# meyerls/FruitNeRF

Measured on AMD Instinct MI355X. Metric: train rays/sec, fruit_nerf on synthetic apple 800x800, higher is better.
Workload: dtype f32 fwd (MLP GEMMs: 3-piece bf16 split, 6 products, ~2^-24) / 2-piece bwd (dX, dW: 3 products, ~2^-17; its forward recompute 3-piece); everything else f32

## Files before the change

### fruitnerf_amd/csrc/hash_scatter.hip

```cpp
#include <stdlib.h>
#include <string.h>

#include "hash_sources.hpp"
#include "sequencer.hpp"

namespace fnr {

constexpr int SC_MAX_ROWS = 8192;
constexpr int SC_MAX_BINS = 256;
constexpr int SC_CHUNK = 512;
constexpr int SC_EMIT_THREADS = 512;
constexpr int SC_PER_THREAD = SC_CHUNK / SC_EMIT_THREADS;
constexpr int SC_BINS_PER_THREAD = 1;
static_assert(SC_MAX_BINS <= SC_EMIT_THREADS, "one bin per thread");
constexpr int SC_CNT_STRIDE = 32;

__device__ unsigned long long g_scatter_overflow_records;
__device__ unsigned long long g_scatter_records[2][64][16];



struct ScatterPlan {
  int log2_rows;
  int bins_per_level;
  long long cap;
  size_t count_bytes, queue_bytes;
  size_t value_bytes;
};

static ScatterPlan scatter_plan(long long N, int n_levels, int log2_T) {
  ScatterPlan p;
  int log2_rows = log2_T - 5;
  if (log2_rows > 13) log2_rows = 13;
  if (log2_rows < 0) log2_rows = 0;
  p.log2_rows = log2_rows;
  p.bins_per_level = 1 << (log2_T - log2_rows);
  const long long avg = (N * 8 + p.bins_per_level - 1) / p.bins_per_level;
  p.cap = (3 * avg + 1023) / 1024 * 1024;
  if (p.cap < 1024) p.cap = 1024;
  const size_t nbins = (size_t)n_levels * p.bins_per_level;
  p.count_bytes = (nbins + 2 * (size_t)n_levels) * SC_CNT_STRIDE * sizeof(unsigned);
  p.value_bytes = nbins * (size_t)p.cap * sizeof(float2);
  p.queue_bytes = p.value_bytes + (nbins * (size_t)p.cap * sizeof(unsigned short) + 255) / 256 * 256;
  return p;
}

__device__ __forceinline__ GridLevel corner_weights(const float (&x)[3], int scaling, uint32_t mask, uint32_t (&h)[8],
                                                    float (&wgt)[8]) {
  GridLevel g = grid_cell(x, scaling);
  grid_corners(g, mask, h);
  const float ox = g.o[0], oy = g.o[1], oz = g.o[2];
  const float mx = 1.0f - ox, my = 1.0f - oy, mz = 1.0f - oz;
  wgt[0] = ox * oy * oz;
  wgt[1] = ox * my * oz;
  wgt[2] = mx * my * oz;
  wgt[3] = mx * oy * oz;
  wgt[4] = ox * oy * mz;
  wgt[5] = ox * my * mz;
  wgt[6] = mx * my * mz;
  wgt[7] = mx * oy * mz;
  return g;
}

template <int CTRL, int ROW_MASK = 0xf>
__device__ __forceinline__ uint32_t dpp_u32(uint32_t old, uint32_t v) {
  return (uint32_t)__builtin_amdgcn_update_dpp((int)old, (int)v, CTRL, ROW_MASK, 0xf, false);
}
template <int CTRL, int ROW_MASK = 0xf>
__device__ __forceinline__ float dpp_f32(float old, float v) {
  return __builtin_bit_cast(float, __builtin_amdgcn_update_dpp(__builtin_bit_cast(int, old), __builtin_bit_cast(int, v),
                                                                 CTRL, ROW_MASK, 0xf, false));
}

struct RunMasks {
  float g1, g2, g4, g8;
  bool tail;
  bool any_run;
};
template <int CTRL>
__device__ __forceinline__ float dpp_shr0_f32(float v) {
  return __builtin_bit_cast(float, __builtin_amdgcn_update_dpp(0, __builtin_bit_cast(int, v), CTRL, 0xf, 0xf, true));
}
__device__ __forceinline__ RunMasks run_structure(uint32_t key_a, uint32_t key_b, int lane) {
  const int j = lane & 15;
  const uint32_t pa = dpp_u32<0x111>(~key_a, key_a), pb = dpp_u32<0x111>(key_b, key_b);
  const bool head = (pa != key_a) || (pb != key_b);
  const unsigned long long heads = __ballot(head);
  const uint32_t row = (uint32_t)(heads >> (lane & 48)) & 0xffffu;
  const uint32_t below = row & ((2u << j) - 1u);
  const int dist = j - (31 - __clz((int)below));
  RunMasks m;
  m.g1 = dist >= 1 ? 1.0f : 0.0f;
  m.g2 = dist >= 2 ? 1.0f : 0.0f;
  m.g4 = dist >= 4 ? 1.0f : 0.0f;
  m.g8 = dist >= 8 ? 1.0f : 0.0f;
  m.tail = (j == 15) || ((row >> (j + 1)) & 1u);
  m.any_run = ~heads != 0ull;
  return m;
}
__device__ __forceinline__ float run_sum(float v, const RunMasks& m) {
  v = fmaf(m.g1, dpp_shr0_f32<0x111>(v), v);
  v = fmaf(m.g2, dpp_shr0_f32<0x112>(v), v);
  v = fmaf(m.g4, dpp_shr0_f32<0x114>(v), v);
  v = fmaf(m.g8, dpp_shr0_f32<0x118>(v), v);
  return v;
}



template <class Source, bool PAIRS>
__global__ __launch_bounds__(SC_EMIT_THREADS) void k_scatter_emit(GridDev grid, Warp warp, Source src, long long N,
                                                      const float2* __restrict__ d_feats, float2* __restrict__ queue_v,
                                                      unsigned short* __restrict__ queue_r, unsigned* __restrict__ qcount, unsigned* __restrict__ qmax,
                                                      long long cap, int log2_rows, int level0, int level_count, int lpb
                                                      ) {
  __shared__ float2 s_val[SC_CHUNK * 8];
  __shared__ unsigned s_key[SC_CHUNK * 8];
  __shared__ unsigned s_cnt[SC_MAX_BINS];
  __shared__ unsigned s_off[SC_MAX_BINS];
  __shared__ unsigned s_base[SC_MAX_BINS];
  __shared__ unsigned s_max;
  __shared__ unsigned s_wsum[SC_EMIT_THREADS / 64];
  const int bins = 1 << (grid.log2_T - log2_rows);
  const int lane = threadIdx.x & 63, wave = threadIdx.x >> 6;
  const uint32_t mask = (1u << grid.log2_T) - 1u;
  const uint32_t row_mask = (1u << log2_rows) - 1u;
  const long long n0 = (long long)blockIdx.x * SC_CHUNK;
  static_assert(SC_PER_THREAD == 1, "one sample per thread");
  const long long n = n0 + threadIdx.x;
  const bool valid = n < N;
  float x[3] = {0.f, 0.f, 0.f};
  float2 gf_next = make_float2(0.f, 0.f);
  const int lrel0 = blockIdx.y * lpb;
  if (valid) {
    gf_next = ntc_load<NT_DFEATS_LD>(&d_feats[(size_t)(level0 + lrel0) * N + n]);
    float px, py, pz;
    src.position(n, px, py, pz);
    warp_position(warp, px, py, pz, x);
  }
  for (int li = 0; li < lpb && lrel0 + li < level_count; ++li) {
  const int lrel = lrel0 + li;
  const int level = level0 + lrel;
  for (int i = threadIdx.x; i < bins; i += SC_EMIT_THREADS) {
    s_cnt[i] = 0;
  }
  if (threadIdx.x == 0) s_max = 0;
  __syncthreads();
  const int scaling = grid.scalings[level];
  const float2 gf = gf_next;
  if (valid && li + 1 < lpb && lrel + 1 < level_count) gf_next = ntc_load<NT_DFEATS_LD>(&d_feats[(size_t)(level + 1) * N + n]);

  uint32_t hk[SC_PER_THREAD][8];
  float vxk[SC_PER_THREAD][8], vyk[SC_PER_THREAD][8];
  float tmax = 0.0f;
  unsigned emit_mask[SC_PER_THREAD];
#pragma unroll
  for (int q = 0; q < SC_PER_THREAD; ++q) {
    float wgt[8];
    const GridLevel g = corner_weights(x, scaling, mask, hk[q], wgt);
    const uint32_t key_a = valid ? (g.f[0] | (g.f[1] << 16)) : 0xffffffffu;
    const uint32_t key_b = valid ? (g.f[2] | ((g.c[0] - g.f[0]) << 16) | ((g.c[1] - g.f[1]) << 17) |
                                    ((g.c[2] - g.f[2]) << 18))
                                 : (0x80000000u | (uint32_t)lane);
    const RunMasks rm = run_structure(key_a, key_b, lane);
    emit_mask[q] = 0;
#pragma unroll
    for (int k = 0; k < 8; ++k) {
      vxk[q][k] = valid ? wgt[k] * gf.x : 0.0f;
      vyk[q][k] = valid ? wgt[k] * gf.y : 0.0f;
    }
    if (rm.any_run) {
#pragma unroll
      for (int k = 0; k < 8; ++k) {
        vxk[q][k] = run_sum(vxk[q][k], rm);
        vyk[q][k] = run_sum(vyk[q][k], rm);
      }
    }
#pragma unroll
    for (int k = 0; k < 8; ++k) {
      if (rm.tail && (vxk[q][k] != 0.0f || vyk[q][k] != 0.0f)) {
        emit_mask[q] |= 1u << k;
        tmax = fmaxf(tmax, fmaxf(fabsf(vxk[q][k]), fabsf(vyk[q][k])));
      }
    }
    if constexpr (PAIRS) {
#pragma unroll
      for (int pr = 0; pr < 4; ++pr) {
        const int ka = (pr == 0) ? 0 : (pr == 1) ? 1 : (pr == 2) ? 4 : 5, kb = (pr == 0) ? 3 : (pr == 1) ? 2 : (pr == 2) ? 7 : 6;
        const unsigned cnt = ((emit_mask[q] >> ka) & 1u) + ((emit_mask[q] >> kb) & 1u);
        if (cnt) atomicAdd(&s_cnt[hk[q][ka] >> log2_rows], cnt);
      }
    } else {
#pragma unroll
      for (int k = 0; k < 8; ++k)
        if ((emit_mask[q] >> k) & 1u) atomicAdd(&s_cnt[hk[q][k] >> log2_rows], 1u);
    }
  }
#pragma unroll
  for (int dsh = 32; dsh >= 1; dsh >>= 1) tmax = fmaxf(tmax, __shfl_xor(tmax, dsh, 64));
  if (lane == 0 && tmax > 0.0f) atomicMax(&s_max, __float_as_uint(tmax));
  __syncthreads();
  if (threadIdx.x == 0 && s_max != 0u) atomicMax(&qmax[(size_t)lrel * SC_CNT_STRIDE], s_max);
  unsigned c4[SC_BINS_PER_THREAD], tsum = 0;
#pragma unroll
  for (int t = 0; t < SC_BINS_PER_THREAD; ++t) {
    const int i = threadIdx.x * SC_BINS_PER_THREAD + t;
    c4[t] = (i < bins) ? s_cnt[i] : 0u;
    tsum += c4[t];
  }
  unsigned incl = tsum;
#pragma unroll
  for (int d = 1; d < 64; d <<= 1) {
    const unsigned u = __shfl_up(incl, d, 64);
    if (lane >= d) incl += u;
  }
  if (lane == 63) s_wsum[wave] = incl;
  __syncthreads();
  unsigned woff = 0;
  for (int w = 0; w < wave; ++w) woff += s_wsum[w];
  unsigned total = 0;
#pragma unroll
  for (int w = 0; w < SC_EMIT_THREADS / 64; ++w) total += s_wsum[w];
  unsigned run = woff + incl - tsum;
#pragma unroll
  for (int t = 0; t < SC_BINS_PER_THREAD; ++t) {
    const int i = threadIdx.x * SC_BINS_PER_THREAD + t;
    if (i < bins) {
      s_off[i] = run;
      s_base[i] = c4[t] ? atomicAdd(&qcount[(size_t)(lrel * bins + i) * SC_CNT_STRIDE], c4[t]) : 0u;
      s_cnt[i] = 0;
      run += c4[t];
    }
  }
  __syncthreads();
#pragma unroll
  for (int q = 0; q < SC_PER_THREAD; ++q) {
    if constexpr (PAIRS) {
#pragma unroll
      for (int pr = 0; pr < 4; ++pr) {
        const int ka = (pr == 0) ? 0 : (pr == 1) ? 1 : (pr == 2) ? 4 : 5, kb = (pr == 0) ? 3 : (pr == 1) ? 2 : (pr == 2) ? 7 : 6;
        const unsigned ea = (emit_mask[q] >> ka) & 1u, eb = (emit_mask[q] >> kb) & 1u;
        if (ea + eb) {
          const unsigned bin = hk[q][ka] >> log2_rows;
          const unsigned pos = s_off[bin] + atomicAdd(&s_cnt[bin], ea + eb);
          if (ea) {
            s_val[pos] = make_float2(vxk[q][ka], vyk[q][ka]);
            s_key[pos] = (hk[q][ka] & row_mask) | (bin << 16);
          }
          if (eb) {
            s_val[pos + ea] = make_float2(vxk[q][kb], vyk[q][kb]);
            s_key[pos + ea] = (hk[q][kb] & row_mask) | (bin << 16);
          }
        }
      }
    } else {
#pragma unroll
      for (int k = 0; k < 8; ++k) {
        if ((emit_mask[q] >> k) & 1u) {
          const int bin = hk[q][k] >> log2_rows;
          const unsigned pos = s_off[bin] + atomicAdd(&s_cnt[bin], 1u);
          s_val[pos] = make_float2(vxk[q][k], vyk[q][k]);
          s_key[pos] = (hk[q][k] & row_mask) | ((unsigned)bin << 16);
        }
      }
    }
  }
  __syncthreads();
  float* table = reinterpret_cast<float*>(grid.table + ((size_t)level << grid.log2_T));
  unsigned overflowed_here = 0;
  for (unsigned i = threadIdx.x; i < total; i += SC_EMIT_THREADS) {
    const float2 v = s_val[i];
    const unsigned key = s_key[i];
    const unsigned bin = key >> 16, row_in_bin = key & 0xffffu;
    const unsigned slot = s_base[bin] + (i - s_off[bin]);
    if ((long long)slot < cap) {
      const size_t q = ((size_t)lrel * bins + bin) * cap + slot;
      queue_v[q] = v;
      queue_r[q] = (unsigned short)row_in_bin;
    } else {
      qmax[(size_t)lrel * SC_CNT_STRIDE + 1] = 1u;
      ++overflowed_here;
      const size_t row = ((size_t)bin << log2_rows) + row_in_bin;
      atomicAdd(table + 2 * row, v.x);
      atomicAdd(table + 2 * row + 1, v.y);
    }
  }
  if (overflowed_here) atomicAdd(&g_scatter_overflow_records, (unsigned long long)overflowed_here);
  __syncthreads();
  }
}

__device__ __forceinline__ void acc_record(unsigned long long* __restrict__ s_acc, unsigned row, const float2& v,
                                           double scale) {
  const long long ix = __double2ll_rn((double)v.x * scale), iy = __double2ll_rn((double)v.y * scale);
  atomicAdd(&s_acc[2 * row], (unsigned long long)ix);
  atomicAdd(&s_acc[2 * row + 1], (unsigned long long)iy);
}

struct AccArgs {
  GridDev grid;
  const float2* queue_v;
  const unsigned short* queue_r;
  unsigned *qcount, *qmax, *qdone;
  long long cap;
  int log2_rows, level0, nbins;
  int kind;
  TableAdam adam;
};

template <bool ADAM>
__device__ __forceinline__ void accumulate_bin(const AccArgs& A, int vblock, unsigned long long* __restrict__ s_acc) {
  const GridDev& grid = A.grid;
  const float2* __restrict__ queue_v = A.queue_v;
  const unsigned short* __restrict__ queue_r = A.queue_r;
  unsigned* __restrict__ qcount = A.qcount;
  unsigned* __restrict__ qmax = A.qmax;
  unsigned* __restrict__ qdone = A.qdone;
  const long long cap = A.cap;
  const int log2_rows = A.log2_rows, level0 = A.level0;
  const TableAdam& adam = A.adam;
  const int rows = 1 << log2_rows;
  const int bins = 1 << (grid.log2_T - log2_rows);
  const int gbin = A.nbins - 1 - vblock;
  const int lrel = gbin / bins, bin = gbin - lrel * bins;
  const int level = level0 + lrel;
  long long n = qcount[(size_t)gbin * SC_CNT_STRIDE];
  const float vmax = __uint_as_float(qmax[(size_t)lrel * SC_CNT_STRIDE]);
  const bool overflowed = qmax[(size_t)lrel * SC_CNT_STRIDE + 1] != 0u;
  {
    const unsigned held_n = (unsigned)n, held_max = __float_as_uint(vmax), held_ovf = overflowed ? 1u : 0u;
    asm volatile("s_waitcnt vmcnt(0) lgkmcnt(0)" ::"v"(held_n), "v"(held_max), "v"(held_ovf) : "memory");
  }
  __syncthreads();
  if (threadIdx.x == 0) {
    qcount[(size_t)gbin * SC_CNT_STRIDE] = 0u;
    if (atomicAdd(&qdone[(size_t)lrel * SC_CNT_STRIDE], 1u) == (unsigned)bins - 1u) {
      qmax[(size_t)lrel * SC_CNT_STRIDE] = 0u;
      qmax[(size_t)lrel * SC_CNT_STRIDE + 1] = 0u;
      qdone[(size_t)lrel * SC_CNT_STRIDE] = 0u;
    }
  }
  const bool have = n != 0 && vmax > 0.0f;
  if (threadIdx.x == 0 && n > 0)
    atomicAdd(&g_scatter_records[A.kind & 1][vblock & 63][0], (unsigned long long)(n > cap ? cap : n));
  if (!ADAM && !have) return;
  if (n > cap) n = cap;
  if (n < 1) n = 1;
  int e;
  (void)frexpf(vmax, &e);
  const int nb = 64 - __clzll((unsigned long long)n);
  int S = 62 - nb - e;
  if (S > 1000) S = 1000;
  const double scale = ldexp(1.0, S), inv = ldexp(1.0, -S);
  for (int i = threadIdx.x; i < 2 * rows; i += blockDim.x) s_acc[i] = 0ull;
  __syncthreads();
  if (!have) n = 0;
  const float2* qv = queue_v + (size_t)gbin * cap;
  const unsigned short* qr = queue_r + (size_t)gbin * cap;
  const float4* qv2 = reinterpret_cast<const float4*>(qv);
  const ushort2* qr2 = reinterpret_cast<const ushort2*>(qr);
  const long long np = n >> 1;
  long long i = threadIdx.x;
  for (; i + 3 * (long long)blockDim.x < np; i += 4 * (long long)blockDim.x) {
    float4 v[4];
    ushort2 row[4];
#pragma unroll
    for (int u = 0; u < 4; ++u) {
      v[u] = ntc_load<NT_QUEUE_LD>(&qv2[i + u * (long long)blockDim.x]);
      row[u] = ntc_load<NT_QUEUE_LD>(&qr2[i + u * (long long)blockDim.x]);
    }
#pragma unroll
    for (int u = 0; u < 4; ++u) {
      acc_record(s_acc, row[u].x, make_float2(v[u].x, v[u].y), scale);
      acc_record(s_acc, row[u].y, make_float2(v[u].z, v[u].w), scale);
    }
  }
  for (; i < np; i += blockDim.x) {
    const float4 v = ntc_load<NT_QUEUE_LD>(&qv2[i]);
    const ushort2 row = ntc_load<NT_QUEUE_LD>(&qr2[i]);
    acc_record(s_acc, row.x, make_float2(v.x, v.y), scale);
    acc_record(s_acc, row.y, make_float2(v.z, v.w), scale);
  }
  if ((n & 1) && threadIdx.x == 0) {
    acc_record(s_acc, qr[n - 1], qv[n - 1], scale);
  }
  __syncthreads();
  float2* dst = grid.table + ((size_t)level << grid.log2_T) + (size_t)bin * rows;
  if constexpr (ADAM) {
    const size_t row0 = ((size_t)level << grid.log2_T) + (size_t)bin * rows;
    const bool wide = rows >= 2 && (((uintptr_t)(adam.p + row0) | (uintptr_t)(adam.m + row0) | (uintptr_t)(adam.v + row0)) & 15u) == 0 &&
                      !overflowed;
    if (wide) {
      float4* P4 = reinterpret_cast<float4*>(adam.p + row0);
      float4* M4 = reinterpret_cast<float4*>(adam.m + row0);
      float4* V4 = reinterpret_cast<float4*>(adam.v + row0);
      unsigned* tw = (adam.touched && rows >= 64) ? adam.touched + (row0 >> 6) : nullptr;
      for (int e4 = threadIdx.x; e4 < (rows >> 1); e4 += blockDim.x) {
        const long long a0 = (long long)s_acc[4 * e4], a1 = (long long)s_acc[4 * e4 + 1],
                        a2 = (long long)s_acc[4 * e4 + 2], a3 = (long long)s_acc[4 * e4 + 3];
        if (tw) {
          const bool now = (a0 | a1 | a2 | a3) != 0;
          const bool ever = (tw[e4 >> 5] >> (e4 & 31)) & 1u;
          if (!now && !ever) continue;
          if (!ever) atomicOr(&tw[e4 >> 5], 1u << (e4 & 31));
        }
        float4 P = P4[e4], M = ntc_load<NT_MOMENT_LD>(&M4[e4]), V = ntc_load<NT_MOMENT_LD>(&V4[e4]);
        const float g0 = (a0 != 0 || a1 != 0) ? 0.0f + (float)((double)a0 * inv) : 0.0f;
        const float g1 = (a0 != 0 || a1 != 0) ? 0.0f + (float)((double)a1 * inv) : 0.0f;
        const float g2 = (a2 != 0 || a3 != 0) ? 0.0f + (float)((double)a2 * inv) : 0.0f;
        const float g3 = (a2 != 0 || a3 != 0) ? 0.0f + (float)((double)a3 * inv) : 0.0f;
        table_adam_update(adam, g0, P.x, M.x, V.x);
        table_adam_update(adam, g1, P.y, M.y, V.y);
        table_adam_update(adam, g2, P.z, M.z, V.z);
        table_adam_update(adam, g3, P.w, M.w, V.w);
        P4[e4] = P;
        ntc_store<NT_MOMENT_ST>(&M4[e4], M);
        ntc_store<NT_MOMENT_ST>(&V4[e4], V);
      }
      return;
    }
    unsigned* tw1 = (adam.touched && rows >= 64) ? adam.touched + (row0 >> 6) : nullptr;
    for (int e2 = threadIdx.x; e2 < rows; e2 += blockDim.x) {
      const long long ax = (long long)s_acc[2 * e2], ay = (long long)s_acc[2 * e2 + 1];
      float2 g = make_float2(0.0f, 0.0f);
      if (overflowed) {
        g = dst[e2];
        if (g.x != 0.0f || g.y != 0.0f) dst[e2] = make_float2(0.0f, 0.0f);
      }
      if (ax != 0 || ay != 0) {
        g.x += (float)((double)ax * inv);
        g.y += (float)((double)ay * inv);
      }
      if (tw1 && (ax != 0 || ay != 0 || g.x != 0.0f || g.y != 0.0f)) {
        const int pair = e2 >> 1;
        if (!((tw1[pair >> 5] >> (pair & 31)) & 1u)) atomicOr(&tw1[pair >> 5], 1u << (pair & 31));
      }
      float2 P = adam.p[row0 + e2], M = adam.m[row0 + e2], V = adam.v[row0 + e2];
      table_adam_update(adam, g.x, P.x, M.x, V.x);
      table_adam_update(adam, g.y, P.y, M.y, V.y);
      adam.p[row0 + e2] = P;
      adam.m[row0 + e2] = M;
      adam.v[row0 + e2] = V;
    }
  } else {
    for (int e2 = threadIdx.x; e2 < rows; e2 += blockDim.x) {
      const long long ax = (long long)s_acc[2 * e2], ay = (long long)s_acc[2 * e2 + 1];
      if (ax != 0 || ay != 0) {
        float2 t = dst[e2];
        t.x += (float)((double)ax * inv);
        t.y += (float)((double)ay * inv);
        dst[e2] = t;
      }
    }
  }
}

extern __shared__ __attribute__((aligned(16))) unsigned char acc_smem[];
template <bool ADAM>
__global__ __launch_bounds__(1024) void k_scatter_accumulate(AccArgs a) {
  accumulate_bin<ADAM>(a, (int)blockIdx.x, reinterpret_cast<unsigned long long*>(acc_smem));
}
template <bool ADAM>
__global__ __launch_bounds__(1024) void k_scatter_accumulate2(AccArgs a, AccArgs b) {
  unsigned long long* s_acc = reinterpret_cast<unsigned long long*>(acc_smem);
  if ((int)blockIdx.x < a.nbins) accumulate_bin<ADAM>(a, (int)blockIdx.x, s_acc);
  else accumulate_bin<ADAM>(b, (int)blockIdx.x - a.nbins, s_acc);
}


template <class Source>
static int scatter_emit(const fnr_grid* grid_grad, const Warp& warp, const Source& src, long long N,
                        const float2* d_feats, int level0, int level_count, void* workspace, size_t workspace_bytes,
                        int workspace_clean, hipStream_t st, const TableAdam* adam, AccArgs& acc) {
  FNR_CHECK_ARG(level0 >= 0 && level_count >= 1 && level0 + level_count <= grid_grad->n_levels,
                "hash scatter: level range [%d,+%d) outside the %d levels", level0, level_count, grid_grad->n_levels);
  const ScatterPlan p = scatter_plan(N, level_count, grid_grad->log2_hashmap_size);
  FNR_CHECK_ARG(p.bins_per_level <= SC_MAX_BINS, "hash scatter: log2_hashmap_size %d too large for the bin histogram",
                grid_grad->log2_hashmap_size);
  FNR_CHECK_ARG(workspace && workspace_bytes >= p.count_bytes + p.queue_bytes, "hash scatter: workspace too small");
  unsigned* qcount = reinterpret_cast<unsigned*>(workspace);
  float2* queue_v = reinterpret_cast<float2*>(reinterpret_cast<char*>(workspace) + p.count_bytes);
  unsigned short* queue_r = reinterpret_cast<unsigned short*>(reinterpret_cast<char*>(workspace) + p.count_bytes + p.value_bytes);
  if (!workspace_clean) FNR_HIP(hipMemsetAsync(qcount, 0, p.count_bytes, st));
  const size_t nbins_all = (size_t)level_count * p.bins_per_level;
  const long long chunks = (N + SC_CHUNK - 1) / SC_CHUNK;
  FNR_CHECK_ARG(chunks < (1ll << 31), "hash scatter: too many samples");
  const GridDev gd = make_grid(grid_grad);
  for (int l = 0; l < grid_grad->n_levels; ++l)
    FNR_CHECK_ARG(gd.scalings[l] > 0 && gd.scalings[l] < 65535, "hash scatter: level resolution %d out of range", gd.scalings[l]);
  bool pairs = true;
  for (int l = level0; l < level0 + level_count; ++l) pairs = pairs && gd.scalings[l] < (1 << p.log2_rows);
  int lpb = 1;
  {
    const char* e = getenv("FNR_EMIT_LPB");
    const int forced = e ? atoi(e) : 0;
    const long long slots = 3ll * device_cu_count();
    while (lpb < level_count && lpb < 8 && chunks * ((level_count + 2 * lpb - 1) / (2 * lpb)) >= 2 * slots) lpb *= 2;
    if (forced > 0) lpb = forced;
    if (lpb > level_count) lpb = level_count;
  }
  const unsigned gy = (unsigned)((level_count + lpb - 1) / lpb);
  if (chunks == 0) {
  } else if (pairs)
    hipLaunchKernelGGL((k_scatter_emit<Source, true>), dim3((unsigned)chunks, gy), dim3(SC_EMIT_THREADS),
                       0, st, gd, warp, src, N, d_feats, queue_v, queue_r, qcount, qcount + nbins_all * SC_CNT_STRIDE, p.cap,
                       p.log2_rows, level0, level_count, lpb);
  else
    hipLaunchKernelGGL((k_scatter_emit<Source, false>), dim3((unsigned)chunks, gy), dim3(SC_EMIT_THREADS),
                       0, st, gd, warp, src, N, d_feats, queue_v, queue_r, qcount, qcount + nbins_all * SC_CNT_STRIDE, p.cap,
                       p.log2_rows, level0, level_count, lpb);
  FNR_LAUNCH_CHECK();
  acc.grid = gd;
  acc.queue_v = queue_v, acc.queue_r = queue_r, acc.qcount = qcount;
  acc.qmax = qcount + nbins_all * SC_CNT_STRIDE;
  acc.qdone = qcount + (nbins_all + level_count) * SC_CNT_STRIDE;
  acc.cap = p.cap, acc.log2_rows = p.log2_rows, acc.level0 = level0;
  acc.nbins = level_count * p.bins_per_level;
  acc.kind = 0;
  acc.adam = adam ? *adam : TableAdam{};
  return FNR_OK;
}

static int acc_lds_bytes(const AccArgs& a) { return (2 << a.log2_rows) * (int)sizeof(unsigned long long); }

static int scatter_accumulate(const AccArgs& a, bool adam, hipStream_t st) {
  const int bytes = acc_lds_bytes(a);
  if (adam) {
    const int rc = ensure_dyn_lds<k_scatter_accumulate<true>>(2 * SC_MAX_ROWS * (int)sizeof(unsigned long long));
    if (rc) return rc;
    hipLaunchKernelGGL(k_scatter_accumulate<true>, dim3((unsigned)a.nbins), dim3(1024), bytes, st, a);
  } else {
    const int rc = ensure_dyn_lds<k_scatter_accumulate<false>>(2 * SC_MAX_ROWS * (int)sizeof(unsigned long long));
    if (rc) return rc;
    hipLaunchKernelGGL(k_scatter_accumulate<false>, dim3((unsigned)a.nbins), dim3(1024), bytes, st, a);
  }
  FNR_LAUNCH_CHECK();
  return FNR_OK;
}

static int scatter_accumulate2(const AccArgs& a, const AccArgs& b, bool adam, hipStream_t st) {
  const int bytes = acc_lds_bytes(a) > acc_lds_bytes(b) ? acc_lds_bytes(a) : acc_lds_bytes(b);
  if (adam) {
    const int rc = ensure_dyn_lds<k_scatter_accumulate2<true>>(2 * SC_MAX_ROWS * (int)sizeof(unsigned long long));
    if (rc) return rc;
    hipLaunchKernelGGL(k_scatter_accumulate2<true>, dim3((unsigned)(a.nbins + b.nbins)), dim3(1024), bytes, st, a, b);
  } else {
    const int rc = ensure_dyn_lds<k_scatter_accumulate2<false>>(2 * SC_MAX_ROWS * (int)sizeof(unsigned long long));
    if (rc) return rc;
    hipLaunchKernelGGL(k_scatter_accumulate2<false>, dim3((unsigned)(a.nbins + b.nbins)), dim3(1024), bytes, st, a, b);
  }
  FNR_LAUNCH_CHECK();
  return FNR_OK;
}

template <class Source>
static int binned_scatter(const fnr_grid* grid_grad, const Warp& warp, const Source& src, long long N,
                          const float2* d_feats, int level0, int level_count, void* workspace, size_t workspace_bytes,
                          int workspace_clean, hipStream_t st, const TableAdam* adam = nullptr) {
  AccArgs acc;
  const int rc = scatter_emit(grid_grad, warp, src, N, d_feats, level0, level_count, workspace, workspace_bytes,
                              workspace_clean, st, adam, acc);
  if (rc) return rc;
  return scatter_accumulate(acc, adam != nullptr, st);
}

constexpr int PROP_PART = 320;

template <int L, int H, bool POSGRAD>
__global__ __launch_bounds__(256) void k_prop_bwd(GridDev grid, float4* __restrict__ d_xw, Warp warp, RaySource src,
                                                  long long N, const float* __restrict__ w0,
                                                  const float* __restrict__ b0, const float* __restrict__ w1,
                                                  const float* __restrict__ b1, const float2* __restrict__ feat_save,
                                                  const float* __restrict__ d_density, float2* __restrict__ d_feats,
                                                  float* __restrict__ partials) {
  constexpr int K = 2 * L;
  __shared__ float s_dh[256][H + 1];
  __shared__ float s_ha[256][H + 1];
  __shared__ float s_f[256][K + 1];
  __shared__ float s_do[256];
  static_assert(H == 16 && K <= 16, "phase 2 is a single 16x16 MFMA tile");
  using f32x4 = __attribute__((ext_vector_type(4))) float;
  const int tid = threadIdx.x;
  const int lane = tid & 63, wave = tid >> 6;
  const int j = lane & 15, g = lane >> 4;
  f32x4 d1 = {0.f, 0.f, 0.f, 0.f}, d2 = {0.f, 0.f, 0.f, 0.f}, d3 = {0.f, 0.f, 0.f, 0.f};
  float db1 = 0.0f;
  const float ones_col0 = (j == 0) ? 1.0f : 0.0f;
  const long long n_iter = (N + 255) / 256;
  for (long long it = blockIdx.x; it < n_iter; it += gridDim.x) {
    const long long n = it * 256 + tid;
    float f[K], dout = 0.0f;
#pragma unroll
    for (int k = 0; k < K; ++k) f[k] = 0.0f;
    bool sel = false;
    float x[3] = {0.f, 0.f, 0.f};
    if (n < N) {
      float px, py, pz;
      src.position(n, px, py, pz);
      sel = warp_position(warp, px, py, pz, x);
#pragma unroll
      for (int l = 0; l < L; ++l) {
        const float2 v = ntc_load<NT_PROP_FEATS>(&feat_save[(size_t)l * N + n]);
        f[2 * l] = v.x;
        f[2 * l + 1] = v.y;
      }
    }
    float a[H];
    float out = b1[0];
#pragma unroll
    for (int o = 0; o < H; ++o) {
      float t = b0[o];
#pragma unroll
      for (int k = 0; k < K; ++k) t = fmaf(w0[o * K + k], f[k], t);
      a[o] = t;
      out = fmaf(w1[o], fmaxf(t, 0.0f), out);
    }
    if (n < N && sel) dout = d_density[n] * expf(fminf(fmaxf(out, -15.0f), 15.0f));
    float df[K];
#pragma unroll
    for (int k = 0; k < K; ++k) df[k] = 0.0f;
#pragma unroll
    for (int o = 0; o < H; ++o) {
      const float dh = (a[o] > 0.0f) ? dout * w1[o] : 0.0f;
      s_dh[tid][o] = dh;
      s_ha[tid][o] = fmaxf(a[o], 0.0f) * dout;
#pragma unroll
      for (int k = 0; k < K; ++k) df[k] = fmaf(dh, w0[o * K + k], df[k]);
    }
#pragma unroll
    for (int k = 0; k < K; ++k) s_f[tid][k] = f[k];
    db1 += dout;
    if (n < N) {
#pragma unroll
      for (int l = 0; l < L; ++l) ntc_store<NT_PROP_DFEATS_ST>(&d_feats[(size_t)l * N + n], make_float2(df[2 * l], df[2 * l + 1]));
    }
    if constexpr (POSGRAD) {
      if (n < N) {
        const uint32_t hmask = (1u << grid.log2_T) - 1u;
        float gx = 0.0f, gy = 0.0f, gz = 0.0f;
#pragma unroll
        for (int l = 0; l < L; ++l) {
          const int scaling = grid.scalings[l];
          const GridLevel gl = grid_cell(x, scaling);
          uint32_t hh[8];
          grid_corners(gl, hmask, hh);
          const float2* lt = grid.table + ((size_t)l << grid.log2_T);
          float dk[8];
#pragma unroll
          for (int k = 0; k < 8; ++k) {
            const float2 v = lt[hh[k]];
            dk[k] = fmaf(df[2 * l], v.x, df[2 * l + 1] * v.y);
          }
          const float ox = gl.o[0], oy = gl.o[1], oz = gl.o[2];
          const float mx = 1.0f - ox, my = 1.0f - oy, mz = 1.0f - oz;
          const float s = sel ? (float)scaling : 0.0f;
          gx += s * (oz * (oy * (dk[0] - dk[3]) + my * (dk[1] - dk[2])) + mz * (oy * (dk[4] - dk[7]) + my * (dk[5] - dk[6])));
          gy += s * (oz * (ox * (dk[0] - dk[1]) + mx * (dk[3] - dk[2])) + mz * (ox * (dk[4] - dk[5]) + mx * (dk[7] - dk[6])));
          gz += s * (oy * (ox * (dk[0] - dk[4]) + mx * (dk[3] - dk[7])) + my * (ox * (dk[1] - dk[5]) + mx * (dk[2] - dk[6])));
        }
        d_xw[n] = make_float4(gx, gy, gz, 0.0f);
      }
    }
    __syncthreads();
    const int row0 = 64 * wave + g;
#pragma unroll 4
    for (int st = 0; st < 16; ++st) {
      const int row = row0 + 4 * st;
      const float a1 = s_dh[row][j], a2 = s_ha[row][j];
      const float bf = (j < K) ? s_f[row][j < K ? j : 0] : 0.0f;
      d1 = __builtin_amdgcn_mfma_f32_16x16x4f32(a1, bf, d1, 0, 0, 0);
      d2 = __builtin_amdgcn_mfma_f32_16x16x4f32(a2, ones_col0, d2, 0, 0, 0);
      d3 = __builtin_amdgcn_mfma_f32_16x16x4f32(a1, ones_col0, d3, 0, 0, 0);
    }
    __syncthreads();
  }
  float* red = &s_dh[0][0];
#pragma unroll
  for (int r = 0; r < 4; ++r) {
    red[((wave * 3 + 0) * 16 + 4 * g + r) * 16 + j] = d1[r];
    red[((wave * 3 + 1) * 16 + 4 * g + r) * 16 + j] = d2[r];
    red[((wave * 3 + 2) * 16 + 4 * g + r) * 16 + j] = d3[r];
  }
  db1 = wave_sum(db1);
  if (lane == 0) s_do[wave] = db1;
  __syncthreads();
  {
    const int o = tid >> 4, k = tid & 15;
    auto total = [&](int which) {
      return (red[((0 * 3 + which) * 16 + o) * 16 + k] + red[((1 * 3 + which) * 16 + o) * 16 + k]) +
             (red[((2 * 3 + which) * 16 + o) * 16 + k] + red[((3 * 3 + which) * 16 + o) * 16 + k]);
    };
    float* part = partials + (size_t)blockIdx.x * PROP_PART;
    part[tid] = total(0);
    if (k == 0) {
      part[256 + o] = total(1);
      part[272 + o] = total(2);
    }
    if (tid == 0) part[288] = (s_do[0] + s_do[1]) + (s_do[2] + s_do[3]);
  }
}

constexpr int PRD_E = 16, PRD_Y = 64;
struct PropReduceArgs {
  const float* partials;
  int nblocks, K;
  float *g_w0, *g_b0, *g_w1, *g_b1;
  WeightAdam wa;
};
template <bool ADAM>
__device__ __forceinline__ void prop_reduce_block(int block, const PropReduceArgs& a) {
  __shared__ float s_part[PRD_Y][PRD_E];
  const float* __restrict__ partials = a.partials;
  const int nblocks = a.nblocks, K = a.K;
  const int t = threadIdx.x % PRD_E, y = threadIdx.x / PRD_E;
  const int e = block * PRD_E + t;
  float s = 0.0f;
  if (e <= 288) {
    int b = y;
    for (; b + 7 * PRD_Y < nblocks; b += 8 * PRD_Y) {
      float v[8];
#pragma unroll
      for (int u = 0; u < 8; ++u) v[u] = partials[(size_t)(b + u * PRD_Y) * PROP_PART + e];
#pragma unroll
      for (int u = 0; u < 8; ++u) s += v[u];
    }
    for (; b < nblocks; b += PRD_Y) s += partials[(size_t)b * PROP_PART + e];
  }
  s_part[y][t] = s;
  __syncthreads();
  if (y != 0 || e > 288) return;
#pragma unroll 8
  for (int q = 1; q < PRD_Y; ++q) s += s_part[q][t];
  if (!ADAM && s == 0.0f) return;
  float* dst = nullptr;
  if (e < 256) {
    const int o = e >> 4, k = e & 15;
    if (k < K) dst = &a.g_w0[o * K + k];
  } else if (e < 272) {
    dst = &a.g_w1[e - 256];
  } else if (e < 288) {
    dst = &a.g_b0[e - 272];
  } else {
    dst = &a.g_b1[0];
  }
  if (!dst) return;
  if constexpr (ADAM) weight_adam_entry(a.wa, dst, s);
  else *dst += s;
}
template <bool ADAM>
__global__ __launch_bounds__(PRD_E * PRD_Y) void k_prop_reduce(PropReduceArgs a) {
  prop_reduce_block<ADAM>((int)blockIdx.x, a);
}
template <bool ADAM>
__global__ __launch_bounds__(PRD_E * PRD_Y) void k_prop_reduce2(PropReduceArgs a, PropReduceArgs b) {
  constexpr int NB = PROP_PART / PRD_E;
  if ((int)blockIdx.x < NB) prop_reduce_block<ADAM>((int)blockIdx.x, a);
  else prop_reduce_block<ADAM>((int)blockIdx.x - NB, b);
}

}

using namespace fnr;


extern "C" int fnr_debug_scatter_overflows(uint64_t* count_host, int reset) {
  FNR_CHECK_ARG(count_host, "debug_scatter_overflows: null argument");
  unsigned long long n = 0;
  FNR_HIP(hipMemcpyFromSymbol(&n, HIP_SYMBOL(g_scatter_overflow_records), sizeof(n)));
  *count_host = n;
  if (reset) {
    n = 0;
    FNR_HIP(hipMemcpyToSymbol(HIP_SYMBOL(g_scatter_overflow_records), &n, sizeof(n)));
  }
  return FNR_OK;
}

extern "C" int fnr_debug_scatter_records(uint64_t* records_host, int reset) {
  FNR_CHECK_ARG(records_host, "debug_scatter_records: null argument");
  FNR_HIP(hipDeviceSynchronize());
  unsigned long long host[2][64][16];
  FNR_HIP(hipMemcpyFromSymbol(host, HIP_SYMBOL(g_scatter_records), sizeof(host)));
  for (int k = 0; k < 2; ++k) {
    records_host[k] = 0;
    for (int i = 0; i < 64; ++i) records_host[k] += host[k][i][0];
  }
  if (reset) {
    memset(host, 0, sizeof(host));
    FNR_HIP(hipMemcpyToSymbol(HIP_SYMBOL(g_scatter_records), host, sizeof(host)));
  }
  return FNR_OK;
}


extern "C" size_t fnr_hash_scatter_workspace_bytes(int64_t n_samples, int n_levels, int log2_hashmap_size) {
  const ScatterPlan p = scatter_plan(n_samples, n_levels, log2_hashmap_size);
  return p.count_bytes + p.queue_bytes;
}

extern "C" int fnr_hash_encode_bwd(const fnr_grid* grid_grad, const fnr_warp* warp, const fnr_rays* rays,
                                   const float* euclid_bins, int S, const float* d_feats, int level_begin,
                                   int level_count, void* workspace, size_t workspace_bytes, int workspace_clean,
                                   void* stream) {
  FNR_SEQ_UNRECORDABLE("fnr_hash_encode_bwd");
  FNR_CHECK_ARG(grid_grad && warp && rays && euclid_bins && d_feats && S > 0, "hash_encode_bwd: null argument");
  FNR_CHECK_ARG(grid_grad->n_levels >= 1 && grid_grad->n_levels <= FNR_MAX_LEVELS, "hash_encode_bwd: n_levels");
  const long long N = rays->n_rays * (long long)S;
  if (N == 0) return FNR_OK;
  RaySource src{make_rays(rays), euclid_bins, S};
  FNR_PROF(OP_ENCODE_BWD, N);
  return binned_scatter(grid_grad, make_warp(warp), src, N, reinterpret_cast<const float2*>(d_feats), level_begin,
                        level_count, workspace, workspace_bytes, workspace_clean, as_stream(stream));
}

extern "C" int fnr_hash_encode_bwd_adam(const fnr_grid* grid_grad, const fnr_warp* warp, const fnr_rays* rays,
                                        const float* euclid_bins, int S, const float* d_feats, void* workspace,
                                        size_t workspace_bytes, int workspace_clean, const fnr_table_adam* adam,
                                        void* stream) {
  if (seq::recording() && grid_grad && warp && rays && adam) {
    const fnr_grid grid_ = *grid_grad;
    const fnr_warp warp_ = *warp;
    const fnr_rays rays_ = *rays;
    const fnr_table_adam adam_ = *adam;
    seq::push("fnr_hash_encode_bwd_adam", [=](const fnr_step_scalars* sc) {
      const fnr_table_adam a = seq::patched(adam_, sc);
      return fnr_hash_encode_bwd_adam(&grid_, &warp_, &rays_, euclid_bins, S, d_feats, workspace, workspace_bytes,
                                      workspace_clean, &a, stream);
    });
  }
  FNR_CHECK_ARG(grid_grad && warp && rays && euclid_bins && d_feats && S > 0, "hash_encode_bwd_adam: null argument");
  FNR_CHECK_ARG(grid_grad->n_levels >= 1 && grid_grad->n_levels <= FNR_MAX_LEVELS, "hash_encode_bwd_adam: n_levels");
  TableAdam t;
  const int rc = make_table_adam(adam, t);
  if (rc) return rc;
  const long long N = rays->n_rays * (long long)S;
  RaySource src{make_rays(rays), euclid_bins, S};
  FNR_PROF(OP_ENCODE_BWD, N);
  return binned_scatter(grid_grad, make_warp(warp), src, N, reinterpret_cast<const float2*>(d_feats), 0,
                        grid_grad->n_levels, workspace, workspace_bytes, workspace_clean, as_stream(stream), &t);
}

extern "C" size_t fnr_prop_density_bwd_workspace_bytes(int64_t n_samples, int n_levels, int log2_hashmap_size) {
  const size_t dfeat = ((size_t)n_levels * (size_t)n_samples * sizeof(float2) + 255) / 256 * 256;
  const size_t partials = (size_t)3 * device_cu_count() * PROP_PART * sizeof(float);
  return dfeat + partials + fnr_hash_scatter_workspace_bytes(n_samples, n_levels, log2_hashmap_size);
}

static int prop_density_bwd_entry(const fnr_prop_net* net, const fnr_prop_net* grads, const fnr_warp* warp,
                                    const fnr_rays* rays, const float* euclid_bins, int S, const float* feat_save,
                                    const float* d_density, float* d_position, void* workspace,
                                    size_t workspace_bytes, int workspace_clean, void* stream,
                                    const fnr_table_adam* table_adam, const fnr_table_adam* weight_adam,
                                    const float* grad_arena, AccArgs* defer_acc = nullptr, int phase = 0,
                                    bool own_scope = true, PropReduceArgs* defer_reduce = nullptr) {
  FNR_CHECK_ARG(net && grads && warp && rays && euclid_bins && feat_save && d_density && workspace && S > 0,
                "prop_density_bwd: null argument");
  WeightAdam wa{};
  TableAdam ta;
  if (table_adam) {
    FNR_CHECK_ARG(weight_adam && grad_arena, "prop_density_bwd_adam: weight_adam / grad_arena missing");
    int rca = make_table_adam(weight_adam, wa.t);
    if (rca) return rca;
    wa.p_off = weight_adam->params - grad_arena;
    wa.m_off = weight_adam->exp_avg - grad_arena;
    wa.v_off = weight_adam->exp_avg_sq - grad_arena;
    rca = make_table_adam(table_adam, ta);
    if (rca) return rca;
  }
  FNR_UNSUPPORTED(net->hidden_dim == 16, "prop_density_bwd: hidden_dim %d not built (16 only)", net->hidden_dim);
  FNR_CHECK_ARG(grads->grid.table && grads->w0 && grads->b0 && grads->w1 && grads->b1,
                "prop_density_bwd: null gradient pointer");
  const long long N = rays->n_rays * (long long)S;
  if (N == 0) return FNR_OK;
  const int L = net->grid.n_levels;
  FNR_CHECK_ARG(workspace_bytes >= fnr_prop_density_bwd_workspace_bytes(N, L, net->grid.log2_hashmap_size),
                "prop_density_bwd: workspace too small");
  RaySource src{make_rays(rays), euclid_bins, S};
  long long blocks = (N + 255) / 256;
  const long long max_blocks = 3ll * device_cu_count();
  if (blocks > max_blocks) blocks = max_blocks;
  {
    static const int cap_per_cu = [] { const char* e = getenv("FNR_PROP_BWD_WGS_PER_CU"); const int v = e ? atoi(e) : 0; return (v >= 1 && v <= 3) ? v : 3; }();
    const long long capped = (long long)cap_per_cu * device_cu_count();
    if (blocks > capped) blocks = capped;
  }
  Warp w = make_warp(warp);
  const float2* fs = reinterpret_cast<const float2*>(feat_save);
  float2* d_feats = reinterpret_cast<float2*>(workspace);
  const size_t dfeat_bytes = ((size_t)L * (size_t)N * sizeof(float2) + 255) / 256 * 256;
  float* partials = reinterpret_cast<float*>(reinterpret_cast<char*>(workspace) + dfeat_bytes);
  const size_t partial_bytes = (size_t)max_blocks * PROP_PART * sizeof(float);
  ::fnr::ProfScope prof_scope__(own_scope ? (int)OP_PROP_BWD : -1, N, stream);
  if (phase != 2) {
  const GridDev pgrid = make_grid(&net->grid);
  float4* d_xw = reinterpret_cast<float4*>(d_position);
#define FNR_PROPB_CASE(LL)                                                                                          \
  case LL:                                                                                                          \
    if (d_xw)                                                                                                       \
      hipLaunchKernelGGL((k_prop_bwd<LL, 16, true>), dim3((unsigned)blocks), dim3(256), 0, as_stream(stream), pgrid, \
                         d_xw, w, src, N, net->w0, net->b0, net->w1, net->b1, fs, d_density, d_feats, partials);    \
    else                                                                                                            \
      hipLaunchKernelGGL((k_prop_bwd<LL, 16, false>), dim3((unsigned)blocks), dim3(256), 0, as_stream(stream), pgrid, \
                         d_xw, w, src, N, net->w0, net->b0, net->w1, net->b1, fs, d_density, d_feats, partials);    \
    break;
  switch (L) {
    FNR_PROPB_CASE(1)
    FNR_PROPB_CASE(2)
    FNR_PROPB_CASE(3)
    FNR_PROPB_CASE(4)
    FNR_PROPB_CASE(5)
    FNR_PROPB_CASE(6)
    FNR_PROPB_CASE(7)
    FNR_PROPB_CASE(8)
    default:
      FNR_UNSUPPORTED(false, "prop_density_bwd: n_levels %d not built (1..8)", L);
  }
#undef FNR_PROPB_CASE
  FNR_LAUNCH_CHECK();
  const PropReduceArgs ra{partials, (int)blocks, 2 * L, grads->w0, grads->b0, grads->w1, grads->b1, table_adam ? wa : WeightAdam{}};
  if (defer_reduce) {
    *defer_reduce = ra;
  } else {
    if (table_adam) hipLaunchKernelGGL(k_prop_reduce<true>, dim3(PROP_PART / PRD_E), dim3(PRD_E * PRD_Y), 0, as_stream(stream), ra);
    else hipLaunchKernelGGL(k_prop_reduce<false>, dim3(PROP_PART / PRD_E), dim3(PRD_E * PRD_Y), 0, as_stream(stream), ra);
    FNR_LAUNCH_CHECK();
  }
  }
  if (phase == 1) return FNR_OK;
  AccArgs acc;
  const int rce = scatter_emit(&grads->grid, w, src, N, d_feats, 0, L,
                               reinterpret_cast<char*>(workspace) + dfeat_bytes + partial_bytes,
                               workspace_bytes - dfeat_bytes - partial_bytes, workspace_clean, as_stream(stream),
                               table_adam ? &ta : nullptr, acc);
  if (rce) return rce;
  acc.kind = 1;
  if (defer_acc) {
    *defer_acc = acc;
    return FNR_OK;
  }
  return scatter_accumulate(acc, table_adam != nullptr, as_stream(stream));
}

extern "C" int fnr_prop_density_bwd(const fnr_prop_net* net, const fnr_prop_net* grads, const fnr_warp* warp,
                                    const fnr_rays* rays, const float* euclid_bins, int S, const float* feat_save,
                                    const float* d_density, float* d_position, void* workspace,
                                    size_t workspace_bytes, int workspace_clean, void* stream) {
  FNR_SEQ_UNRECORDABLE("fnr_prop_density_bwd");
  return prop_density_bwd_entry(net, grads, warp, rays, euclid_bins, S, feat_save, d_density, d_position, workspace,
                                workspace_bytes, workspace_clean, stream, nullptr, nullptr, nullptr);
}

extern "C" int fnr_prop_density_bwd_adam(const fnr_prop_net* net, const fnr_prop_net* grads, const fnr_warp* warp,
                                         const fnr_rays* rays, const float* euclid_bins, int S, const float* feat_save,
                                         const float* d_density, float* d_position, const fnr_table_adam* table_adam,
                                         const fnr_table_adam* weight_adam, const float* grad_arena, void* workspace,
                                         size_t workspace_bytes, int workspace_clean, void* stream) {
  FNR_SEQ_UNRECORDABLE("fnr_prop_density_bwd_adam");
  FNR_CHECK_ARG(table_adam && weight_adam && grad_arena, "prop_density_bwd_adam: optimiser descriptors missing");
  return prop_density_bwd_entry(net, grads, warp, rays, euclid_bins, S, feat_save, d_density, d_position, workspace,
                                workspace_bytes, workspace_clean, stream, table_adam, weight_adam, grad_arena);
}

extern "C" int fnr_prop_density_bwd_pair(const fnr_prop_net* const* nets, const fnr_prop_net* const* grads,
                                         const fnr_warp* const* warps, const fnr_rays* rays,
                                         const float* const* euclid_bins, const int* S, const float* const* feat_save,
                                         const float* const* d_density, float* const* d_position,
                                         const fnr_table_adam* const* table_adam, const fnr_table_adam* weight_adam,
                                         const float* grad_arena, void* const* workspace, const size_t* workspace_bytes,
                                         const int* workspace_clean, void* stream) {
  if (seq::recording() && nets && grads && warps && rays && euclid_bins && S && feat_save && d_density && d_position &&
      workspace && workspace_bytes && workspace_clean && nets[0] && nets[1] && grads[0] && grads[1] && warps[0] && warps[1]) {
    struct Pair {
      fnr_prop_net net[2], grad[2];
      fnr_warp warp[2];
      fnr_rays rays;
      const float* euclid[2];
      int S[2];
      const float* feat[2];
      const float* dd[2];
      float* dpos[2];
      fnr_table_adam tadam[2], wadam;
      bool has_adam;
      void* ws[2];
      size_t ws_bytes[2];
      int ws_clean[2];
    } p;
    for (int q = 0; q < 2; ++q) {
      p.net[q] = *nets[q], p.grad[q] = *grads[q], p.warp[q] = *warps[q], p.euclid[q] = euclid_bins[q], p.S[q] = S[q];
      p.feat[q] = feat_save[q], p.dd[q] = d_density[q], p.dpos[q] = d_position[q], p.ws[q] = workspace[q];
      p.ws_bytes[q] = workspace_bytes[q], p.ws_clean[q] = workspace_clean[q];
    }
    p.rays = *rays;
    p.has_adam = table_adam && table_adam[0] && table_adam[1] && weight_adam;
    if (p.has_adam) p.tadam[0] = *table_adam[0], p.tadam[1] = *table_adam[1], p.wadam = *weight_adam;
    seq::push("fnr_prop_density_bwd_pair", [=](const fnr_step_scalars* sc) {
      const fnr_prop_net* n_[2] = {&p.net[0], &p.net[1]};
      const fnr_prop_net* g_[2] = {&p.grad[0], &p.grad[1]};
      const fnr_warp* w_[2] = {&p.warp[0], &p.warp[1]};
      const fnr_table_adam t0 = seq::patched(p.tadam[0], sc), t1 = seq::patched(p.tadam[1], sc), wa = seq::patched(p.wadam, sc);
      const fnr_table_adam* t_[2] = {&t0, &t1};
      return fnr_prop_density_bwd_pair(n_, g_, w_, &p.rays, p.euclid, p.S, p.feat, p.dd, p.dpos, p.has_adam ? t_ : nullptr,
                      p.has_adam ? &wa : nullptr, grad_arena, p.ws, p.ws_bytes, p.ws_clean, stream);
    });
  }
  FNR_CHECK_ARG(nets && grads && warps && rays && euclid_bins && S && feat_save && d_density && d_position && workspace &&
                    workspace_bytes && workspace_clean,
                "prop_density_bwd_pair: null argument");
  FNR_CHECK_ARG(nets[0] != nets[1] && grads[0] != grads[1] && workspace[0] != workspace[1],
                "prop_density_bwd_pair: the two levels must have their own network, gradients and workspace");
  const bool adam = table_adam && table_adam[0] && table_adam[1];
  FNR_CHECK_ARG(adam || !(table_adam && (table_adam[0] || table_adam[1])), "prop_density_bwd_pair: one table_adam missing");
  if (rays->n_rays == 0) return FNR_OK;
  FNR_PROF(OP_PROP_BWD, rays->n_rays * ((long long)S[0] + (long long)S[1]));
  AccArgs acc[2];
  for (int q = 0; q < 2; ++q) {
    const int rc = prop_density_bwd_entry(nets[q], grads[q], warps[q], rays, euclid_bins[q], S[q], feat_save[q], d_density[q],
                                          d_position[q], workspace[q], workspace_bytes[q], workspace_clean[q], stream,
                                          adam ? table_adam[q] : nullptr, adam ? weight_adam : nullptr,
                                          adam ? grad_arena : nullptr, &acc[q], 0, false);
    if (rc) return rc;
  }
  const bool first_longer = (long long)S[0] >= (long long)S[1];
  return scatter_accumulate2(first_longer ? acc[0] : acc[1], first_longer ? acc[1] : acc[0], adam, as_stream(stream));
}

extern "C" int fnr_prop_density_bwd_pair_split(const fnr_prop_net* const* nets, const fnr_prop_net* const* grads,
                                               const fnr_warp* const* warps, const fnr_rays* rays,
                                               const float* const* euclid_bins, const int* S, const float* const* feat_save,
                                               const float* const* d_density, float* const* d_position,
                                               const fnr_table_adam* const* table_adam, const fnr_table_adam* weight_adam,
                                               const float* grad_arena, void* const* workspace, const size_t* workspace_bytes,
                                               const int* workspace_clean, void* stream, void* position_ready_event) {
  if (seq::recording() && nets && grads && warps && rays && euclid_bins && S && feat_save && d_density && d_position &&
      workspace && workspace_bytes && workspace_clean && nets[0] && nets[1] && grads[0] && grads[1] && warps[0] && warps[1]) {
    struct Pair {
      fnr_prop_net net[2], grad[2];
      fnr_warp warp[2];
      fnr_rays rays;
      const float* euclid[2];
      int S[2];
      const float* feat[2];
      const float* dd[2];
      float* dpos[2];
      fnr_table_adam tadam[2], wadam;
      bool has_adam;
      void* ws[2];
      size_t ws_bytes[2];
      int ws_clean[2];
    } p;
    for (int q = 0; q < 2; ++q) {
      p.net[q] = *nets[q], p.grad[q] = *grads[q], p.warp[q] = *warps[q], p.euclid[q] = euclid_bins[q], p.S[q] = S[q];
      p.feat[q] = feat_save[q], p.dd[q] = d_density[q], p.dpos[q] = d_position[q], p.ws[q] = workspace[q];
      p.ws_bytes[q] = workspace_bytes[q], p.ws_clean[q] = workspace_clean[q];
    }
    p.rays = *rays;
    p.has_adam = table_adam && table_adam[0] && table_adam[1] && weight_adam;
    if (p.has_adam) p.tadam[0] = *table_adam[0], p.tadam[1] = *table_adam[1], p.wadam = *weight_adam;
    seq::push("fnr_prop_density_bwd_pair_split", [=](const fnr_step_scalars* sc) {
      const fnr_prop_net* n_[2] = {&p.net[0], &p.net[1]};
      const fnr_prop_net* g_[2] = {&p.grad[0], &p.grad[1]};
      const fnr_warp* w_[2] = {&p.warp[0], &p.warp[1]};
      const fnr_table_adam t0 = seq::patched(p.tadam[0], sc), t1 = seq::patched(p.tadam[1], sc), wa = seq::patched(p.wadam, sc);
      const fnr_table_adam* t_[2] = {&t0, &t1};
      return fnr_prop_density_bwd_pair_split(n_, g_, w_, &p.rays, p.euclid, p.S, p.feat, p.dd, p.dpos, p.has_adam ? t_ : nullptr,
                      p.has_adam ? &wa : nullptr, grad_arena, p.ws, p.ws_bytes, p.ws_clean, stream, position_ready_event);
    });
  }
  FNR_CHECK_ARG(nets && grads && warps && rays && euclid_bins && S && feat_save && d_density && d_position && workspace &&
                    workspace_bytes && workspace_clean,
                "prop_density_bwd_pair_split: null argument");
  FNR_CHECK_ARG(nets[0] != nets[1] && grads[0] != grads[1] && workspace[0] != workspace[1],
                "prop_density_bwd_pair_split: the two levels must have their own network, gradients and workspace");
  const bool adam = table_adam && table_adam[0] && table_adam[1];
  FNR_CHECK_ARG(adam || !(table_adam && (table_adam[0] || table_adam[1])), "prop_density_bwd_pair_split: one table_adam missing");
  if (rays->n_rays == 0) {
    if (position_ready_event) FNR_HIP(hipEventRecord(reinterpret_cast<hipEvent_t>(position_ready_event), as_stream(stream)));
    return FNR_OK;
  }
  FNR_PROF(OP_PROP_BWD, rays->n_rays * ((long long)S[0] + (long long)S[1]));
  AccArgs acc[2];
  PropReduceArgs red[2];
  for (int phase = 1; phase <= 2; ++phase) {
    for (int q = 0; q < 2; ++q) {
      const int rc = prop_density_bwd_entry(nets[q], grads[q], warps[q], rays, euclid_bins[q], S[q], feat_save[q], d_density[q],
                                            d_position[q], workspace[q], workspace_bytes[q], workspace_clean[q], stream,
                                            adam ? table_adam[q] : nullptr, adam ? weight_adam : nullptr,
                                            adam ? grad_arena : nullptr, &acc[q], phase, false, phase == 1 ? &red[q] : nullptr);
      if (rc) return rc;
    }
    if (phase == 1) {
      if (position_ready_event) FNR_HIP(hipEventRecord(reinterpret_cast<hipEvent_t>(position_ready_event), as_stream(stream)));
      constexpr unsigned NB = PROP_PART / PRD_E;
      if (adam) hipLaunchKernelGGL(k_prop_reduce2<true>, dim3(2 * NB), dim3(PRD_E * PRD_Y), 0, as_stream(stream), red[0], red[1]);
      else hipLaunchKernelGGL(k_prop_reduce2<false>, dim3(2 * NB), dim3(PRD_E * PRD_Y), 0, as_stream(stream), red[0], red[1]);
      FNR_LAUNCH_CHECK();
    }
  }
  const bool first_longer = (long long)S[0] >= (long long)S[1];
  return scatter_accumulate2(first_longer ? acc[0] : acc[1], first_longer ? acc[1] : acc[0], adam, as_stream(stream));
}
```

Measured before the change: 6.029 million.

## Merge proposal-level backward launches and stage MLP weights in shared memory

The two proposal-network levels now run their backward pass, scatter emit, reduce and accumulate stages as combined launches (emit2, fused accumulate+reduce) instead of separate per-level launches. The per-level phases are restructured into a plan/launch split. The prop backward kernel stages the small MLP weights into LDS and prefetches inputs. It also stores pre-activations in shared memory rather than registers and processes grid levels in a non-unrolled loop to cut register pressure. The aim is fewer launches, less idle tail between small kernels and better occupancy, at the cost of more LDS traffic and added complexity.

```diff
diff --git a/fruitnerf_amd/csrc/hash_scatter.hip b/fruitnerf_amd/csrc/hash_scatter.hip
--- a/fruitnerf_amd/csrc/hash_scatter.hip
+++ b/fruitnerf_amd/csrc/hash_scatter.hip
@@ -108,12 +108,32 @@
 
 
 
+template <class Source>
+struct EmitArgs {
+  GridDev grid;
+  Warp warp;
+  Source src;
+  long long N;
+  const float2* d_feats;
+  float2* queue_v;
+  unsigned short* queue_r;
+  unsigned *qcount, *qmax;
+  long long cap;
+  int log2_rows, level0, level_count, lpb;
+  unsigned chunks, gy;
+};
+
 template <class Source, bool PAIRS>
-__global__ __launch_bounds__(SC_EMIT_THREADS) void k_scatter_emit(GridDev grid, Warp warp, Source src, long long N,
-                                                      const float2* __restrict__ d_feats, float2* __restrict__ queue_v,
-                                                      unsigned short* __restrict__ queue_r, unsigned* __restrict__ qcount, unsigned* __restrict__ qmax,
-                                                      long long cap, int log2_rows, int level0, int level_count, int lpb
-                                                      ) {
+__device__ __forceinline__ void emit_block(const EmitArgs<Source>& A, unsigned bx, unsigned by) {
+  const GridDev& grid = A.grid;
+  const Source& src = A.src;
+  const long long N = A.N, cap = A.cap;
+  const float2* __restrict__ d_feats = A.d_feats;
+  float2* __restrict__ queue_v = A.queue_v;
+  unsigned short* __restrict__ queue_r = A.queue_r;
+  unsigned* __restrict__ qcount = A.qcount;
+  unsigned* __restrict__ qmax = A.qmax;
+  const int log2_rows = A.log2_rows, level0 = A.level0, level_count = A.level_count, lpb = A.lpb;
   __shared__ float2 s_val[SC_CHUNK * 8];
   __shared__ unsigned s_key[SC_CHUNK * 8];
   __shared__ unsigned s_cnt[SC_MAX_BINS];
@@ -125,18 +145,18 @@
   const int lane = threadIdx.x & 63, wave = threadIdx.x >> 6;
   const uint32_t mask = (1u << grid.log2_T) - 1u;
   const uint32_t row_mask = (1u << log2_rows) - 1u;
-  const long long n0 = (long long)blockIdx.x * SC_CHUNK;
+  const long long n0 = (long long)bx * SC_CHUNK;
   static_assert(SC_PER_THREAD == 1, "one sample per thread");
   const long long n = n0 + threadIdx.x;
   const bool valid = n < N;
   float x[3] = {0.f, 0.f, 0.f};
   float2 gf_next = make_float2(0.f, 0.f);
-  const int lrel0 = blockIdx.y * lpb;
+  const int lrel0 = (int)by * lpb;
   if (valid) {
     gf_next = ntc_load<NT_DFEATS_LD>(&d_feats[(size_t)(level0 + lrel0) * N + n]);
     float px, py, pz;
     src.position(n, px, py, pz);
-    warp_position(warp, px, py, pz, x);
+    warp_position(A.warp, px, py, pz, x);
   }
   for (int li = 0; li < lpb && lrel0 + li < level_count; ++li) {
   const int lrel = lrel0 + li;
@@ -287,6 +307,21 @@
   }
   if (overflowed_here) atomicAdd(&g_scatter_overflow_records, (unsigned long long)overflowed_here);
   __syncthreads();
+  }
+}
+
+template <class Source, bool PAIRS>
+__global__ __launch_bounds__(SC_EMIT_THREADS) void k_scatter_emit(EmitArgs<Source> a) {
+  emit_block<Source, PAIRS>(a, blockIdx.x, blockIdx.y);
+}
+template <class Source, bool PAIRS>
+__global__ __launch_bounds__(SC_EMIT_THREADS) void k_scatter_emit2(EmitArgs<Source> a, EmitArgs<Source> b) {
+  const unsigned na = a.chunks * a.gy;
+  if (blockIdx.x < na) {
+    emit_block<Source, PAIRS>(a, blockIdx.x % a.chunks, blockIdx.x / a.chunks);
+  } else {
+    const unsigned v = blockIdx.x - na;
+    emit_block<Source, PAIRS>(b, v % b.chunks, v / b.chunks);
   }
 }
 
@@ -469,9 +504,15 @@
 
 
 template <class Source>
-static int scatter_emit(const fnr_grid* grid_grad, const Warp& warp, const Source& src, long long N,
-                        const float2* d_feats, int level0, int level_count, void* workspace, size_t workspace_bytes,
-                        int workspace_clean, hipStream_t st, const TableAdam* adam, AccArgs& acc) {
+struct EmitPlan {
+  EmitArgs<Source> args;
+  bool pairs;
+  AccArgs acc;
+};
+template <class Source>
+static int scatter_emit_plan(const fnr_grid* grid_grad, const Warp& warp, const Source& src, long long N,
+                             const float2* d_feats, int level0, int level_count, void* workspace, size_t workspace_bytes,
+                             int workspace_clean, hipStream_t st, const TableAdam* adam, EmitPlan<Source>& plan) {
   FNR_CHECK_ARG(level0 >= 0 && level_count >= 1 && level0 + level_count <= grid_grad->n_levels,
                 "hash scatter: level range [%d,+%d) outside the %d levels", level0, level_count, grid_grad->n_levels);
   const ScatterPlan p = scatter_plan(N, level_count, grid_grad->log2_hashmap_size);
@@ -481,13 +522,13 @@
   unsigned* qcount = reinterpret_cast<unsigned*>(workspace);
   float2* queue_v = reinterpret_cast<float2*>(reinterpret_cast<char*>(workspace) + p.count_bytes);
   unsigned short* queue_r = reinterpret_cast<unsigned short*>(reinterpret_cast<char*>(workspace) + p.count_bytes + p.value_bytes);
-  if (!workspace_clean) FNR_HIP(hipMemsetAsync(qcount, 0, p.count_bytes, st));
   const size_t nbins_all = (size_t)level_count * p.bins_per_level;
   const long long chunks = (N + SC_CHUNK - 1) / SC_CHUNK;
   FNR_CHECK_ARG(chunks < (1ll << 31), "hash scatter: too many samples");
   const GridDev gd = make_grid(grid_grad);
   for (int l = 0; l < grid_grad->n_levels; ++l)
     FNR_CHECK_ARG(gd.scalings[l] > 0 && gd.scalings[l] < 65535, "hash scatter: level resolution %d out of range", gd.scalings[l]);
+  if (!workspace_clean) FNR_HIP(hipMemsetAsync(qcount, 0, p.count_bytes, st));
   bool pairs = true;
   for (int l = level0; l < level0 + level_count; ++l) pairs = pairs && gd.scalings[l] < (1 << p.log2_rows);
   int lpb = 1;
@@ -500,16 +541,10 @@
     if (lpb > level_count) lpb = level_count;
   }
   const unsigned gy = (unsigned)((level_count + lpb - 1) / lpb);
-  if (chunks == 0) {
-  } else if (pairs)
-    hipLaunchKernelGGL((k_scatter_emit<Source, true>), dim3((unsigned)chunks, gy), dim3(SC_EMIT_THREADS),
-                       0, st, gd, warp, src, N, d_feats, queue_v, queue_r, qcount, qcount + nbins_all * SC_CNT_STRIDE, p.cap,
-                       p.log2_rows, level0, level_count, lpb);
-  else
-    hipLaunchKernelGGL((k_scatter_emit<Source, false>), dim3((unsigned)chunks, gy), dim3(SC_EMIT_THREADS),
-                       0, st, gd, warp, src, N, d_feats, queue_v, queue_r, qcount, qcount + nbins_all * SC_CNT_STRIDE, p.cap,
-                       p.log2_rows, level0, level_count, lpb);
-  FNR_LAUNCH_CHECK();
+  plan.pairs = pairs;
+  plan.args = EmitArgs<Source>{gd, warp, src, N, d_feats, queue_v, queue_r, qcount, qcount + nbins_all * SC_CNT_STRIDE, p.cap,
+                               p.log2_rows, level0, level_count, lpb, (unsigned)chunks, gy};
+  AccArgs& acc = plan.acc;
   acc.grid = gd;
   acc.queue_v = queue_v, acc.queue_r = queue_r, acc.qcount = qcount;
   acc.qmax = qcount + nbins_all * SC_CNT_STRIDE;
@@ -518,6 +553,34 @@
   acc.nbins = level_count * p.bins_per_level;
   acc.kind = 0;
   acc.adam = adam ? *adam : TableAdam{};
+  return FNR_OK;
+}
+
+template <class Source>
+static int scatter_emit_launch(const EmitPlan<Source>& plan, hipStream_t st) {
+  const EmitArgs<Source>& a = plan.args;
+  if (a.chunks == 0) {
+  } else if (plan.pairs)
+    hipLaunchKernelGGL((k_scatter_emit<Source, true>), dim3(a.chunks, a.gy), dim3(SC_EMIT_THREADS), 0, st, a);
+  else
+    hipLaunchKernelGGL((k_scatter_emit<Source, false>), dim3(a.chunks, a.gy), dim3(SC_EMIT_THREADS), 0, st, a);
+  FNR_LAUNCH_CHECK();
+  return FNR_OK;
+}
+
+template <class Source>
+static int scatter_emit_launch2(const EmitPlan<Source>& a, const EmitPlan<Source>& b, hipStream_t st) {
+  const unsigned long long blocks = (unsigned long long)a.args.chunks * a.args.gy + (unsigned long long)b.args.chunks * b.args.gy;
+  if (a.pairs != b.pairs || a.args.chunks == 0 || b.args.chunks == 0 || blocks >= (1ull << 31)) {
+    const int rc = scatter_emit_launch(a, st);
+    if (rc) return rc;
+    return scatter_emit_launch(b, st);
+  }
+  if (a.pairs)
+    hipLaunchKernelGGL((k_scatter_emit2<Source, true>), dim3((unsigned)blocks), dim3(SC_EMIT_THREADS), 0, st, a.args, b.args);
+  else
+    hipLaunchKernelGGL((k_scatter_emit2<Source, false>), dim3((unsigned)blocks), dim3(SC_EMIT_THREADS), 0, st, a.args, b.args);
+  FNR_LAUNCH_CHECK();
   return FNR_OK;
 }
 
@@ -538,95 +601,113 @@
   return FNR_OK;
 }
 
-static int scatter_accumulate2(const AccArgs& a, const AccArgs& b, bool adam, hipStream_t st) {
-  const int bytes = acc_lds_bytes(a) > acc_lds_bytes(b) ? acc_lds_bytes(a) : acc_lds_bytes(b);
-  if (adam) {
-    const int rc = ensure_dyn_lds<k_scatter_accumulate2<true>>(2 * SC_MAX_ROWS * (int)sizeof(unsigned long long));
-    if (rc) return rc;
-    hipLaunchKernelGGL(k_scatter_accumulate2<true>, dim3((unsigned)(a.nbins + b.nbins)), dim3(1024), bytes, st, a, b);
-  } else {
-    const int rc = ensure_dyn_lds<k_scatter_accumulate2<false>>(2 * SC_MAX_ROWS * (int)sizeof(unsigned long long));
-    if (rc) return rc;
-    hipLaunchKernelGGL(k_scatter_accumulate2<false>, dim3((unsigned)(a.nbins + b.nbins)), dim3(1024), bytes, st, a, b);
-  }
-  FNR_LAUNCH_CHECK();
-  return FNR_OK;
-}
-
 template <class Source>
 static int binned_scatter(const fnr_grid* grid_grad, const Warp& warp, const Source& src, long long N,
                           const float2* d_feats, int level0, int level_count, void* workspace, size_t workspace_bytes,
                           int workspace_clean, hipStream_t st, const TableAdam* adam = nullptr) {
-  AccArgs acc;
-  const int rc = scatter_emit(grid_grad, warp, src, N, d_feats, level0, level_count, workspace, workspace_bytes,
-                              workspace_clean, st, adam, acc);
+  EmitPlan<Source> plan;
+  int rc = scatter_emit_plan(grid_grad, warp, src, N, d_feats, level0, level_count, workspace, workspace_bytes,
+                             workspace_clean, st, adam, plan);
   if (rc) return rc;
-  return scatter_accumulate(acc, adam != nullptr, st);
-}
-
+  rc = scatter_emit_launch(plan, st);
+  if (rc) return rc;
+  return scatter_accumulate(plan.acc, adam != nullptr, st);
+}
+
+constexpr int PROP_BWD_ROWS = 2;
+constexpr int PROP_BWD_PG_LEVELS = 2;
 constexpr int PROP_PART = 320;
 
+struct PropBwdArgs {
+  GridDev grid;
+  float4* d_xw;
+  Warp warp;
+  RaySource src;
+  long long N;
+  const float *w0, *b0, *w1, *b1;
+  const float2* feat_save;
+  const float* d_density;
+  float2* d_feats;
+  float* partials;
+};
+
 template <int L, int H, bool POSGRAD>
-__global__ __launch_bounds__(256) void k_prop_bwd(GridDev grid, float4* __restrict__ d_xw, Warp warp, RaySource src,
-                                                  long long N, const float* __restrict__ w0,
-                                                  const float* __restrict__ b0, const float* __restrict__ w1,
-                                                  const float* __restrict__ b1, const float2* __restrict__ feat_save,
-                                                  const float* __restrict__ d_density, float2* __restrict__ d_feats,
-                                                  float* __restrict__ partials) {
+__device__ __forceinline__ void prop_bwd_body(const PropBwdArgs& A, int wg, int nwg) {
   constexpr int K = 2 * L;
-  __shared__ float s_dh[256][H + 1];
-  __shared__ float s_ha[256][H + 1];
+  constexpr int W_B0 = H * K, W_W1 = W_B0 + H, W_B1 = W_W1 + H, W_N = W_B1 + 1;
+  __shared__ float s_a[256][H + 1];
   __shared__ float s_f[256][K + 1];
   __shared__ float s_do[256];
+  __shared__ __attribute__((aligned(16))) float s_w[(W_N + 3) / 4 * 4];
   static_assert(H == 16 && K <= 16, "phase 2 is a single 16x16 MFMA tile");
+  static_assert(4 * 3 * 16 * 16 <= 256 * (H + 1), "the cross-wave reduction reuses s_a");
   using f32x4 = __attribute__((ext_vector_type(4))) float;
+  const GridDev& grid = A.grid;
+  const RaySource& src = A.src;
+  const long long N = A.N;
+  const float2* __restrict__ feat_save = A.feat_save;
+  const float* __restrict__ d_density = A.d_density;
+  float2* __restrict__ d_feats = A.d_feats;
   const int tid = threadIdx.x;
   const int lane = tid & 63, wave = tid >> 6;
   const int j = lane & 15, g = lane >> 4;
+  for (int i = tid; i < W_N; i += 256)
+    s_w[i] = i < W_B0 ? A.w0[i] : i < W_W1 ? A.b0[i - W_B0] : i < W_B1 ? A.w1[i - W_W1] : A.b1[0];
   f32x4 d1 = {0.f, 0.f, 0.f, 0.f}, d2 = {0.f, 0.f, 0.f, 0.f}, d3 = {0.f, 0.f, 0.f, 0.f};
   float db1 = 0.0f;
   const float ones_col0 = (j == 0) ? 1.0f : 0.0f;
   const long long n_iter = (N + 255) / 256;
-  for (long long it = blockIdx.x; it < n_iter; it += gridDim.x) {
+  struct Inputs {
+    float f[K], dd, px, py, pz;
+  };
+  auto fetch = [&](long long it, Inputs& in) {
+    const long long n = it * 256 + tid;
+#pragma unroll
+    for (int k = 0; k < K; ++k) in.f[k] = 0.0f;
+    in.dd = 0.0f, in.px = 0.0f, in.py = 0.0f, in.pz = 0.0f;
+    if (it < n_iter && n < N) {
+      src.position(n, in.px, in.py, in.pz);
+#pragma unroll
+      for (int l = 0; l < L; ++l) {
+        const float2 v = ntc_load<NT_PROP_FEATS>(&feat_save[(size_t)l * N + n]);
+        in.f[2 * l] = v.x;
+        in.f[2 * l + 1] = v.y;
+      }
+      in.dd = d_density[n];
+    }
+  };
+  Inputs cur;
+  fetch(wg, cur);
+  __syncthreads();
+  const float w1j = s_w[W_W1 + j];
+  for (long long it = wg; it < n_iter; it += nwg) {
     const long long n = it * 256 + tid;
     float f[K], dout = 0.0f;
 #pragma unroll
-    for (int k = 0; k < K; ++k) f[k] = 0.0f;
+    for (int k = 0; k < K; ++k) f[k] = cur.f[k];
     bool sel = false;
     float x[3] = {0.f, 0.f, 0.f};
-    if (n < N) {
-      float px, py, pz;
-      src.position(n, px, py, pz);
-      sel = warp_position(warp, px, py, pz, x);
-#pragma unroll
-      for (int l = 0; l < L; ++l) {
-        const float2 v = ntc_load<NT_PROP_FEATS>(&feat_save[(size_t)l * N + n]);
-        f[2 * l] = v.x;
-        f[2 * l + 1] = v.y;
-      }
-    }
-    float a[H];
-    float out = b1[0];
-#pragma unroll
+    if (n < N) sel = warp_position(A.warp, cur.px, cur.py, cur.pz, x);
+    float out = s_w[W_B1];
+#pragma unroll PROP_BWD_ROWS
     for (int o = 0; o < H; ++o) {
-      float t = b0[o];
-#pragma unroll
-      for (int k = 0; k < K; ++k) t = fmaf(w0[o * K + k], f[k], t);
-      a[o] = t;
-      out = fmaf(w1[o], fmaxf(t, 0.0f), out);
-    }
-    if (n < N && sel) dout = d_density[n] * expf(fminf(fmaxf(out, -15.0f), 15.0f));
+      float t = s_w[W_B0 + o];
+#pragma unroll
+      for (int k = 0; k < K; ++k) t = fmaf(s_w[o * K + k], f[k], t);
+      s_a[tid][o] = t;
+      out = fmaf(s_w[W_W1 + o], fmaxf(t, 0.0f), out);
+    }
+    if (n < N && sel) dout = cur.dd * expf(fminf(fmaxf(out, -15.0f), 15.0f));
     float df[K];
 #pragma unroll
     for (int k = 0; k < K; ++k) df[k] = 0.0f;
-#pragma unroll
+#pragma unroll PROP_BWD_ROWS
     for (int o = 0; o < H; ++o) {
-      const float dh = (a[o] > 0.0f) ? dout * w1[o] : 0.0f;
-      s_dh[tid][o] = dh;
-      s_ha[tid][o] = fmaxf(a[o], 0.0f) * dout;
-#pragma unroll
-      for (int k = 0; k < K; ++k) df[k] = fmaf(dh, w0[o * K + k], df[k]);
-    }
+      const float dh = (s_a[tid][o] > 0.0f) ? dout * s_w[W_W1 + o] : 0.0f;
+#pragma unroll
+      for (int k = 0; k < K; ++k) df[k] = fmaf(dh, s_w[o * K + k], df[k]);
+    }
+    s_do[tid] = dout;
 #pragma unroll
     for (int k = 0; k < K; ++k) s_f[tid][k] = f[k];
     db1 += dout;
@@ -638,35 +719,48 @@
       if (n < N) {
         const uint32_t hmask = (1u << grid.log2_T) - 1u;
         float gx = 0.0f, gy = 0.0f, gz = 0.0f;
-#pragma unroll
-        for (int l = 0; l < L; ++l) {
-          const int scaling = grid.scalings[l];
-          const GridLevel gl = grid_cell(x, scaling);
-          uint32_t hh[8];
-          grid_corners(gl, hmask, hh);
-          const float2* lt = grid.table + ((size_t)l << grid.log2_T);
-          float dk[8];
-#pragma unroll
-          for (int k = 0; k < 8; ++k) {
-            const float2 v = lt[hh[k]];
-            dk[k] = fmaf(df[2 * l], v.x, df[2 * l + 1] * v.y);
+#pragma unroll 1
+        for (int l0 = 0; l0 < L; l0 += PROP_BWD_PG_LEVELS) {
+#pragma unroll
+          for (int u = 0; u < PROP_BWD_PG_LEVELS; ++u) {
+            const int l = l0 + u;
+            if (l >= L) break;
+            float dfx = df[0], dfy = df[1];
+#pragma unroll
+            for (int q = 1; q < L; ++q) {
+              dfx = (l == q) ? df[2 * q] : dfx;
+              dfy = (l == q) ? df[2 * q + 1] : dfy;
+            }
+            const int scaling = grid.scalings[l];
+            const GridLevel gl = grid_cell(x, scaling);
+            uint32_t hh[8];
+            grid_corners(gl, hmask, hh);
+            const float2* lt = grid.table + ((size_t)l << grid.log2_T);
+            float dk[8];
+#pragma unroll
+            for (int k = 0; k < 8; ++k) {
+              const float2 v = lt[hh[k]];
+              dk[k] = fmaf(dfx, v.x, dfy * v.y);
+            }
+            const float ox = gl.o[0], oy = gl.o[1], oz = gl.o[2];
+            const float mx = 1.0f - ox, my = 1.0f - oy, mz = 1.0f - oz;
+            const float s = sel ? (float)scaling : 0.0f;
+            gx += s * (oz * (oy * (dk[0] - dk[3]) + my * (dk[1] - dk[2])) + mz * (oy * (dk[4] - dk[7]) + my * (dk[5] - dk[6])));
+            gy += s * (oz * (ox * (dk[0] - dk[1]) + mx * (dk[3] - dk[2])) + mz * (ox * (dk[4] - dk[5]) + mx * (dk[7] - dk[6])));
+            gz += s * (oy * (ox * (dk[0] - dk[4]) + mx * (dk[3] - dk[7])) + my * (ox * (dk[1] - dk[5]) + mx * (dk[2] - dk[6])));
           }
-          const float ox = gl.o[0], oy = gl.o[1], oz = gl.o[2];
-          const float mx = 1.0f - ox, my = 1.0f - oy, mz = 1.0f - oz;
-          const float s = sel ? (float)scaling : 0.0f;
-          gx += s * (oz * (oy * (dk[0] - dk[3]) + my * (dk[1] - dk[2])) + mz * (oy * (dk[4] - dk[7]) + my * (dk[5] - dk[6])));
-          gy += s * (oz * (ox * (dk[0] - dk[1]) + mx * (dk[3] - dk[2])) + mz * (ox * (dk[4] - dk[5]) + mx * (dk[7] - dk[6])));
-          gz += s * (oy * (ox * (dk[0] - dk[4]) + mx * (dk[3] - dk[7])) + my * (ox * (dk[1] - dk[5]) + mx * (dk[2] - dk[6])));
         }
-        d_xw[n] = make_float4(gx, gy, gz, 0.0f);
+        A.d_xw[n] = make_float4(gx, gy, gz, 0.0f);
       }
     }
+    fetch(it + nwg, cur);
     __syncthreads();
     const int row0 = 64 * wave + g;
 #pragma unroll 4
     for (int st = 0; st < 16; ++st) {
       const int row = row0 + 4 * st;
-      const float a1 = s_dh[row][j], a2 = s_ha[row][j];
+      const float av = s_a[row][j], dv = s_do[row];
+      const float a1 = (av > 0.0f) ? dv * w1j : 0.0f, a2 = fmaxf(av, 0.0f) * dv;
       const float bf = (j < K) ? s_f[row][j < K ? j : 0] : 0.0f;
       d1 = __builtin_amdgcn_mfma_f32_16x16x4f32(a1, bf, d1, 0, 0, 0);
       d2 = __builtin_amdgcn_mfma_f32_16x16x4f32(a2, ones_col0, d2, 0, 0, 0);
@@ -674,7 +768,7 @@
     }
     __syncthreads();
   }
-  float* red = &s_dh[0][0];
+  float* red = &s_a[0][0];
 #pragma unroll
   for (int r = 0; r < 4; ++r) {
     red[((wave * 3 + 0) * 16 + 4 * g + r) * 16 + j] = d1[r];
@@ -690,7 +784,7 @@
       return (red[((0 * 3 + which) * 16 + o) * 16 + k] + red[((1 * 3 + which) * 16 + o) * 16 + k]) +
              (red[((2 * 3 + which) * 16 + o) * 16 + k] + red[((3 * 3 + which) * 16 + o) * 16 + k]);
     };
-    float* part = partials + (size_t)blockIdx.x * PROP_PART;
+    float* part = A.partials + (size_t)wg * PROP_PART;
     part[tid] = total(0);
     if (k == 0) {
       part[256 + o] = total(1);
@@ -698,6 +792,16 @@
     }
     if (tid == 0) part[288] = (s_do[0] + s_do[1]) + (s_do[2] + s_do[3]);
   }
+}
+
+template <int L, int H, bool POSGRAD>
+__global__ __launch_bounds__(256, 4) void k_prop_bwd(PropBwdArgs a) {
+  prop_bwd_body<L, H, POSGRAD>(a, (int)blockIdx.x, (int)gridDim.x);
+}
+template <int L, int H, bool POSGRAD>
+__global__ __launch_bounds__(256, 4) void k_prop_bwd2(PropBwdArgs a, PropBwdArgs b, int na) {
+  if ((int)blockIdx.x < na) prop_bwd_body<L, H, POSGRAD>(a, (int)blockIdx.x, na);
+  else prop_bwd_body<L, H, POSGRAD>(b, (int)blockIdx.x - na, (int)gridDim.x - na);
 }
 
 constexpr int PRD_E = 16, PRD_Y = 64;
@@ -758,6 +862,41 @@
   else prop_reduce_block<ADAM>((int)blockIdx.x - NB, b);
 }
 
+static_assert(PRD_E * PRD_Y == 1024, "the reductions run in the accumulate launch's workgroups");
+template <bool ADAM>
+__global__ __launch_bounds__(1024) void k_scatter_accumulate2_reduce(AccArgs a, AccArgs b, PropReduceArgs ra, PropReduceArgs rb) {
+  constexpr int NB = PROP_PART / PRD_E;
+  unsigned long long* s_acc = reinterpret_cast<unsigned long long*>(acc_smem);
+  const int blk = (int)blockIdx.x, nacc = a.nbins + b.nbins;
+  if (blk < a.nbins) accumulate_bin<ADAM>(a, blk, s_acc);
+  else if (blk < nacc) accumulate_bin<ADAM>(b, blk - a.nbins, s_acc);
+  else if (blk < nacc + NB) prop_reduce_block<ADAM>(blk - nacc, ra);
+  else prop_reduce_block<ADAM>(blk - nacc - NB, rb);
+}
+
+static int scatter_accumulate2_reduce(const AccArgs& a, const AccArgs& b, const PropReduceArgs& ra, const PropReduceArgs& rb,
+                                      bool adam, hipStream_t st) {
+  constexpr unsigned NB = PROP_PART / PRD_E;
+  const int bytes = acc_lds_bytes(a) > acc_lds_bytes(b) ? acc_lds_bytes(a) : acc_lds_bytes(b);
+  const unsigned blocks = (unsigned)(a.nbins + b.nbins) + 2 * NB;
+  if (adam) {
+    const int rc = ensure_dyn_lds<k_scatter_accumulate2_reduce<true>>(2 * SC_MAX_ROWS * (int)sizeof(unsigned long long));
+    if (rc) return rc;
+    hipLaunchKernelGGL(k_scatter_accumulate2_reduce<true>, dim3(blocks), dim3(1024), bytes, st, a, b, ra, rb);
+  } else {
+    const int rc = ensure_dyn_lds<k_scatter_accumulate2_reduce<false>>(2 * SC_MAX_ROWS * (int)sizeof(unsigned long long));
+    if (rc) return rc;
+    hipLaunchKernelGGL(k_scatter_accumulate2_reduce<false>, dim3(blocks), dim3(1024), bytes, st, a, b, ra, rb);
+  }
+  FNR_LAUNCH_CHECK();
+  return FNR_OK;
+}
+
+template __global__ void k_scatter_accumulate2<true>(AccArgs, AccArgs);
+template __global__ void k_scatter_accumulate2<false>(AccArgs, AccArgs);
+template __global__ void k_prop_reduce2<true>(PropReduceArgs, PropReduceArgs);
+template __global__ void k_prop_reduce2<false>(PropReduceArgs, PropReduceArgs);
+
 }
 
 using namespace fnr;
@@ -845,13 +984,20 @@
   return dfeat + partials + fnr_hash_scatter_workspace_bytes(n_samples, n_levels, log2_hashmap_size);
 }
 
-static int prop_density_bwd_entry(const fnr_prop_net* net, const fnr_prop_net* grads, const fnr_warp* warp,
-                                    const fnr_rays* rays, const float* euclid_bins, int S, const float* feat_save,
-                                    const float* d_density, float* d_position, void* workspace,
-                                    size_t workspace_bytes, int workspace_clean, void* stream,
-                                    const fnr_table_adam* table_adam, const fnr_table_adam* weight_adam,
-                                    const float* grad_arena, AccArgs* defer_acc = nullptr, int phase = 0,
-                                    bool own_scope = true, PropReduceArgs* defer_reduce = nullptr) {
+struct PropLevelPlan {
+  PropBwdArgs bwd;
+  int L, blocks;
+  bool posgrad, adam;
+  PropReduceArgs red;
+  EmitPlan<RaySource> emit;
+  long long N;
+};
+
+static int prop_level_plan(const fnr_prop_net* net, const fnr_prop_net* grads, const fnr_warp* warp, const fnr_rays* rays,
+                           const float* euclid_bins, int S, const float* feat_save, const float* d_density,
+                           float* d_position, void* workspace, size_t workspace_bytes, int workspace_clean, void* stream,
+                           const fnr_table_adam* table_adam, const fnr_table_adam* weight_adam, const float* grad_arena,
+                           PropLevelPlan& plan) {
   FNR_CHECK_ARG(net && grads && warp && rays && euclid_bins && feat_save && d_density && workspace && S > 0,
                 "prop_density_bwd: null argument");
   WeightAdam wa{};
@@ -870,8 +1016,10 @@
   FNR_CHECK_ARG(grads->grid.table && grads->w0 && grads->b0 && grads->w1 && grads->b1,
                 "prop_density_bwd: null gradient pointer");
   const long long N = rays->n_rays * (long long)S;
+  plan.N = N;
   if (N == 0) return FNR_OK;
   const int L = net->grid.n_levels;
+  FNR_UNSUPPORTED(L >= 1 && L <= 8, "prop_density_bwd: n_levels %d not built (1..8)", L);
   FNR_CHECK_ARG(workspace_bytes >= fnr_prop_density_bwd_workspace_bytes(N, L, net->grid.log2_hashmap_size),
                 "prop_density_bwd: workspace too small");
   RaySource src{make_rays(rays), euclid_bins, S};
@@ -883,26 +1031,40 @@
     const long long capped = (long long)cap_per_cu * device_cu_count();
     if (blocks > capped) blocks = capped;
   }
-  Warp w = make_warp(warp);
-  const float2* fs = reinterpret_cast<const float2*>(feat_save);
+  const Warp w = make_warp(warp);
   float2* d_feats = reinterpret_cast<float2*>(workspace);
   const size_t dfeat_bytes = ((size_t)L * (size_t)N * sizeof(float2) + 255) / 256 * 256;
   float* partials = reinterpret_cast<float*>(reinterpret_cast<char*>(workspace) + dfeat_bytes);
   const size_t partial_bytes = (size_t)max_blocks * PROP_PART * sizeof(float);
-  ::fnr::ProfScope prof_scope__(own_scope ? (int)OP_PROP_BWD : -1, N, stream);
-  if (phase != 2) {
-  const GridDev pgrid = make_grid(&net->grid);
-  float4* d_xw = reinterpret_cast<float4*>(d_position);
-#define FNR_PROPB_CASE(LL)                                                                                          \
-  case LL:                                                                                                          \
-    if (d_xw)                                                                                                       \
-      hipLaunchKernelGGL((k_prop_bwd<LL, 16, true>), dim3((unsigned)blocks), dim3(256), 0, as_stream(stream), pgrid, \
-                         d_xw, w, src, N, net->w0, net->b0, net->w1, net->b1, fs, d_density, d_feats, partials);    \
-    else                                                                                                            \
-      hipLaunchKernelGGL((k_prop_bwd<LL, 16, false>), dim3((unsigned)blocks), dim3(256), 0, as_stream(stream), pgrid, \
-                         d_xw, w, src, N, net->w0, net->b0, net->w1, net->b1, fs, d_density, d_feats, partials);    \
+  plan.L = L, plan.blocks = (int)blocks, plan.posgrad = d_position != nullptr, plan.adam = table_adam != nullptr;
+  plan.bwd = PropBwdArgs{make_grid(&net->grid), reinterpret_cast<float4*>(d_position), w, src, N, net->w0, net->b0, net->w1,
+                         net->b1, reinterpret_cast<const float2*>(feat_save), d_density, d_feats, partials};
+  plan.red = PropReduceArgs{partials, (int)blocks, 2 * L, grads->w0, grads->b0, grads->w1, grads->b1, table_adam ? wa : WeightAdam{}};
+  const int rce = scatter_emit_plan(&grads->grid, w, src, N, d_feats, 0, L,
+                                    reinterpret_cast<char*>(workspace) + dfeat_bytes + partial_bytes,
+                                    workspace_bytes - dfeat_bytes - partial_bytes, workspace_clean, as_stream(stream),
+                                    table_adam ? &ta : nullptr, plan.emit);
+  if (rce) return rce;
+  plan.emit.acc.kind = 1;
+  return FNR_OK;
+}
+
+static int prop_bwd_launch(const PropLevelPlan& a, const PropLevelPlan* b, hipStream_t st) {
+#define FNR_PROPB_LAUNCH(LL, PG)                                                                                        \
+  if (b)                                                                                                                \
+    hipLaunchKernelGGL((k_prop_bwd2<LL, 16, PG>), dim3((unsigned)(a.blocks + b->blocks)), dim3(256), 0, st, a.bwd, b->bwd, \
+                       a.blocks);                                                                                       \
+  else                                                                                                                  \
+    hipLaunchKernelGGL((k_prop_bwd<LL, 16, PG>), dim3((unsigned)a.blocks), dim3(256), 0, st, a.bwd);
+#define FNR_PROPB_CASE(LL)            \
+  case LL:                            \
+    if (a.posgrad) {                  \
+      FNR_PROPB_LAUNCH(LL, true)      \
+    } else {                          \
+      FNR_PROPB_LAUNCH(LL, false)     \
+    }                                 \
     break;
-  switch (L) {
+  switch (a.L) {
     FNR_PROPB_CASE(1)
     FNR_PROPB_CASE(2)
     FNR_PROPB_CASE(3)
@@ -912,32 +1074,78 @@
     FNR_PROPB_CASE(7)
     FNR_PROPB_CASE(8)
     default:
-      FNR_UNSUPPORTED(false, "prop_density_bwd: n_levels %d not built (1..8)", L);
+      FNR_UNSUPPORTED(false, "prop_density_bwd: n_levels %d not built (1..8)", a.L);
   }
 #undef FNR_PROPB_CASE
+#undef FNR_PROPB_LAUNCH
   FNR_LAUNCH_CHECK();
-  const PropReduceArgs ra{partials, (int)blocks, 2 * L, grads->w0, grads->b0, grads->w1, grads->b1, table_adam ? wa : WeightAdam{}};
-  if (defer_reduce) {
-    *defer_reduce = ra;
+  return FNR_OK;
+}
+
+static int prop_density_bwd_entry(const fnr_prop_net* net, const fnr_prop_net* grads, const fnr_warp* warp,
+                                    const fnr_rays* rays, const float* euclid_bins, int S, const float* feat_save,
+                                    const float* d_density, float* d_position, void* workspace,
+                                    size_t workspace_bytes, int workspace_clean, void* stream,
+                                    const fnr_table_adam* table_adam, const fnr_table_adam* weight_adam,
+                                    const float* grad_arena) {
+  PropLevelPlan plan;
+  int rc = prop_level_plan(net, grads, warp, rays, euclid_bins, S, feat_save, d_density, d_position, workspace, workspace_bytes,
+                           workspace_clean, stream, table_adam, weight_adam, grad_arena, plan);
+  if (rc || plan.N == 0) return rc;
+  ::fnr::ProfScope prof_scope__((int)OP_PROP_BWD, plan.N, stream);
+  hipStream_t st = as_stream(stream);
+  rc = prop_bwd_launch(plan, nullptr, st);
+  if (rc) return rc;
+  if (plan.adam) hipLaunchKernelGGL(k_prop_reduce<true>, dim3(PROP_PART / PRD_E), dim3(PRD_E * PRD_Y), 0, st, plan.red);
+  else hipLaunchKernelGGL(k_prop_reduce<false>, dim3(PROP_PART / PRD_E), dim3(PRD_E * PRD_Y), 0, st, plan.red);
+  FNR_LAUNCH_CHECK();
+  rc = scatter_emit_launch(plan.emit, st);
+  if (rc) return rc;
+  return scatter_accumulate(plan.emit.acc, plan.adam, st);
+}
+
+static int prop_density_bwd_pair_launches(const fnr_prop_net* const* nets, const fnr_prop_net* const* grads,
+                                          const fnr_warp* const* warps, const fnr_rays* rays, const float* const* euclid_bins,
+                                          const int* S, const float* const* feat_save, const float* const* d_density,
+                                          float* const* d_position, const fnr_table_adam* const* table_adam,
+                                          const fnr_table_adam* weight_adam, const float* grad_arena, void* const* workspace,
+                                          const size_t* workspace_bytes, const int* workspace_clean, void* stream,
+                                          void* position_ready_event, const char* who) {
+  FNR_CHECK_ARG(nets && grads && warps && rays && euclid_bins && S && feat_save && d_density && d_position && workspace &&
+                    workspace_bytes && workspace_clean,
+                "%s: null argument", who);
+  FNR_CHECK_ARG(nets[0] != nets[1] && grads[0] != grads[1] && workspace[0] != workspace[1],
+                "%s: the two levels must have their own network, gradients and workspace", who);
+  const bool adam = table_adam && table_adam[0] && table_adam[1];
+  FNR_CHECK_ARG(adam || !(table_adam && (table_adam[0] || table_adam[1])), "%s: one table_adam missing", who);
+  hipStream_t st = as_stream(stream);
+  if (rays->n_rays == 0) {
+    if (position_ready_event) FNR_HIP(hipEventRecord(reinterpret_cast<hipEvent_t>(position_ready_event), st));
+    return FNR_OK;
+  }
+  FNR_PROF(OP_PROP_BWD, rays->n_rays * ((long long)S[0] + (long long)S[1]));
+  PropLevelPlan plan[2];
+  for (int q = 0; q < 2; ++q) {
+    const int rc = prop_level_plan(nets[q], grads[q], warps[q], rays, euclid_bins[q], S[q], feat_save[q], d_density[q],
+                                   d_position[q], workspace[q], workspace_bytes[q], workspace_clean[q], stream,
+                                   adam ? table_adam[q] : nullptr, adam ? weight_adam : nullptr, adam ? grad_arena : nullptr,
+                                   plan[q]);
+    if (rc) return rc;
+  }
+  const int first = (long long)S[0] >= (long long)S[1] ? 0 : 1;
+  const PropLevelPlan &a = plan[first], &b = plan[1 - first];
+  int rc;
+  if (a.L == b.L && a.posgrad == b.posgrad) {
+    rc = prop_bwd_launch(a, &b, st);
   } else {
-    if (table_adam) hipLaunchKernelGGL(k_prop_reduce<true>, dim3(PROP_PART / PRD_E), dim3(PRD_E * PRD_Y), 0, as_stream(stream), ra);
-    else hipLaunchKernelGGL(k_prop_reduce<false>, dim3(PROP_PART / PRD_E), dim3(PRD_E * PRD_Y), 0, as_stream(stream), ra);
-    FNR_LAUNCH_CHECK();
-  }
-  }
-  if (phase == 1) return FNR_OK;
-  AccArgs acc;
-  const int rce = scatter_emit(&grads->grid, w, src, N, d_feats, 0, L,
-                               reinterpret_cast<char*>(workspace) + dfeat_bytes + partial_bytes,
-                               workspace_bytes - dfeat_bytes - partial_bytes, workspace_clean, as_stream(stream),
-                               table_adam ? &ta : nullptr, acc);
-  if (rce) return rce;
-  acc.kind = 1;
-  if (defer_acc) {
-    *defer_acc = acc;
-    return FNR_OK;
-  }
-  return scatter_accumulate(acc, table_adam != nullptr, as_stream(stream));
+    rc = prop_bwd_launch(plan[0], nullptr, st);
+    if (!rc) rc = prop_bwd_launch(plan[1], nullptr, st);
+  }
+  if (rc) return rc;
+  if (position_ready_event) FNR_HIP(hipEventRecord(reinterpret_cast<hipEvent_t>(position_ready_event), st));
+  rc = scatter_emit_launch2(a.emit, b.emit, st);
+  if (rc) return rc;
+  return scatter_accumulate2_reduce(a.emit.acc, b.emit.acc, plan[0].red, plan[1].red, adam, st);
 }
 
 extern "C" int fnr_prop_density_bwd(const fnr_prop_net* net, const fnr_prop_net* grads, const fnr_warp* warp,
@@ -1002,25 +1210,9 @@
                       p.has_adam ? &wa : nullptr, grad_arena, p.ws, p.ws_bytes, p.ws_clean, stream);
     });
   }
-  FNR_CHECK_ARG(nets && grads && warps && rays && euclid_bins && S && feat_save && d_density && d_position && workspace &&
-                    workspace_bytes && workspace_clean,
-                "prop_density_bwd_pair: null argument");
-  FNR_CHECK_ARG(nets[0] != nets[1] && grads[0] != grads[1] && workspace[0] != workspace[1],
-                "prop_density_bwd_pair: the two levels must have their own network, gradients and workspace");
-  const bool adam = table_adam && table_adam[0] && table_adam[1];
-  FNR_CHECK_ARG(adam || !(table_adam && (table_adam[0] || table_adam[1])), "prop_density_bwd_pair: one table_adam missing");
-  if (rays->n_rays == 0) return FNR_OK;
-  FNR_PROF(OP_PROP_BWD, rays->n_rays * ((long long)S[0] + (long long)S[1]));
-  AccArgs acc[2];
-  for (int q = 0; q < 2; ++q) {
-    const int rc = prop_density_bwd_entry(nets[q], grads[q], warps[q], rays, euclid_bins[q], S[q], feat_save[q], d_density[q],
-                                          d_position[q], workspace[q], workspace_bytes[q], workspace_clean[q], stream,
-                                          adam ? table_adam[q] : nullptr, adam ? weight_adam : nullptr,
-                                          adam ? grad_arena : nullptr, &acc[q], 0, false);
-    if (rc) return rc;
-  }
-  const bool first_longer = (long long)S[0] >= (long long)S[1];
-  return scatter_accumulate2(first_longer ? acc[0] : acc[1], first_longer ? acc[1] : acc[0], adam, as_stream(stream));
+  return prop_density_bwd_pair_launches(nets, grads, warps, rays, euclid_bins, S, feat_save, d_density, d_position, table_adam,
+                                        weight_adam, grad_arena, workspace, workspace_bytes, workspace_clean, stream, nullptr,
+                                        "prop_density_bwd_pair");
 }
 
 extern "C" int fnr_prop_density_bwd_pair_split(const fnr_prop_net* const* nets, const fnr_prop_net* const* grads,
@@ -1065,36 +1257,7 @@
                       p.has_adam ? &wa : nullptr, grad_arena, p.ws, p.ws_bytes, p.ws_clean, stream, position_ready_event);
     });
   }
-  FNR_CHECK_ARG(nets && grads && warps && rays && euclid_bins && S && feat_save && d_density && d_position && workspace &&
-                    workspace_bytes && workspace_clean,
-                "prop_density_bwd_pair_split: null argument");
-  FNR_CHECK_ARG(nets[0] != nets[1] && grads[0] != grads[1] && workspace[0] != workspace[1],
-                "prop_density_bwd_pair_split: the two levels must have their own network, gradients and workspace");
-  const bool adam = table_adam && table_adam[0] && table_adam[1];
-  FNR_CHECK_ARG(adam || !(table_adam && (table_adam[0] || table_adam[1])), "prop_density_bwd_pair_split: one table_adam missing");
-  if (rays->n_rays == 0) {
-    if (position_ready_event) FNR_HIP(hipEventRecord(reinterpret_cast<hipEvent_t>(position_ready_event), as_stream(stream)));
-    return FNR_OK;
-  }
-  FNR_PROF(OP_PROP_BWD, rays->n_rays * ((long long)S[0] + (long long)S[1]));
-  AccArgs acc[2];
-  PropReduceArgs red[2];
-  for (int phase = 1; phase <= 2; ++phase) {
-    for (int q = 0; q < 2; ++q) {
-      const int rc = prop_density_bwd_entry(nets[q], grads[q], warps[q], rays, euclid_bins[q], S[q], feat_save[q], d_density[q],
-                                            d_position[q], workspace[q], workspace_bytes[q], workspace_clean[q], stream,
-                                            adam ? table_adam[q] : nullptr, adam ? weight_adam : nullptr,
-                                            adam ? grad_arena : nullptr, &acc[q], phase, false, phase == 1 ? &red[q] : nullptr);
-      if (rc) return rc;
-    }
-    if (phase == 1) {
-      if (position_ready_event) FNR_HIP(hipEventRecord(reinterpret_cast<hipEvent_t>(position_ready_event), as_stream(stream)));
-      constexpr unsigned NB = PROP_PART / PRD_E;
-      if (adam) hipLaunchKernelGGL(k_prop_reduce2<true>, dim3(2 * NB), dim3(PRD_E * PRD_Y), 0, as_stream(stream), red[0], red[1]);
-      else hipLaunchKernelGGL(k_prop_reduce2<false>, dim3(2 * NB), dim3(PRD_E * PRD_Y), 0, as_stream(stream), red[0], red[1]);
-      FNR_LAUNCH_CHECK();
-    }
-  }
-  const bool first_longer = (long long)S[0] >= (long long)S[1];
-  return scatter_accumulate2(first_longer ? acc[0] : acc[1], first_longer ? acc[1] : acc[0], adam, as_stream(stream));
-}
+  return prop_density_bwd_pair_launches(nets, grads, warps, rays, euclid_bins, S, feat_save, d_density, d_position, table_adam,
+                                        weight_adam, grad_arena, workspace, workspace_bytes, workspace_clean, stream, position_ready_event,
+                                        "prop_density_bwd_pair_split");
+}
```

Result: no change. 6.028 million, median of 2 (-0.0%).
